# NVIDIA-RTX/RTXPT

Hardware: AMD Instinct MI355X
Metric: Mrays/s at 4K 4spp 8-bounce bistro-like (extend + shadow rays / wall time of pt_render) (higher is better)
Workload: dtype f32; 1 GPU; C3 bistro-like street canyon, 2808008 triangles, 64 materials, 32 textures 1024^2, 7368 emissive-triangle + env-quad lights, 3840x2160, 4 spp, 8 bounces, NEE 5 candidates + RR, lp types binary16 (reference default), environment cube 2048 BC6H (reference default on D3D12); BVH builder=PLOC + parallel re-insertion + cost-driven wide nodes, built on device, buildMs 78.6 (host part 0.0), 275780 wide n; parallelism=pixel-tile shard x1 + 1 gather, gather=none (1 GPU), transport=none, rehearsal=False

## Files before the change

### include/mi355pt_testhooks.h

```cpp
#ifndef MI355PT_TESTHOOKS_H
#define MI355PT_TESTHOOKS_H
#include "mi355pt.h"
#ifdef __cplusplus
extern "C" {
#endif
int32_t pt_probe(pt_context* ctx, int32_t kind, const void* in, size_t inBytes, void* out, size_t outBytes, uint32_t n);
#ifdef __cplusplus
}
#endif
#endif
```

### rtxpt_amd/__init__.py

```python
import ctypes
import os
import subprocess

import numpy as np

from . import scenes

_HERE = os.path.dirname(os.path.abspath(__file__))
LIB_PATH = os.environ.get("MI355PT_LIB", os.path.join(_HERE, "libmi355pt.so"))
HOOKS_LIB_PATH = os.path.join(_HERE, "libmi355pt_testhooks.so")
_libs = {}

PT_OK = 0
PT_ERROR_INVALID_ARGUMENT, PT_ERROR_NO_DEVICE, PT_ERROR_HIP, PT_ERROR_IO, PT_ERROR_UNSUPPORTED, PT_ERROR_NOT_READY = 1, 2, 3, 4, 5, 6
PT_TEX_RGBA8_UNORM, PT_TEX_RGBA8_SRGB, PT_TEX_RGBA32F = 0, 1, 2
STATUS = {0: "PT_OK", 1: "PT_ERROR_INVALID_ARGUMENT", 2: "PT_ERROR_NO_DEVICE", 3: "PT_ERROR_HIP", 4: "PT_ERROR_IO", 5: "PT_ERROR_UNSUPPORTED", 6: "PT_ERROR_NOT_READY"}

EXPORTS = [
    "pt_create", "pt_destroy", "pt_get_last_error", "pt_load_scene_gltf", "pt_gltf_animation_load", "pt_gltf_animation_instances", "pt_gltf_animation_positions", "pt_gltf_animation_normals", "pt_animate_normals", "pt_gltf_animation_free", "pt_set_geometry", "pt_set_instances", "pt_set_materials",
    "pt_set_environment", "pt_set_environment_cube", "pt_image_read_dds_cube", "pt_set_environment_bake", "pt_set_environment_compression", "pt_set_procedural_sky", "pt_procedural_sky_default_params", "pt_procedural_sky_update", "pt_env_bake_lights", "pt_set_lights", "pt_set_light_importance_boost", "pt_set_local_light_sampling", "pt_get_light_feedback", "pt_set_neeat", "pt_set_view_projection", "pt_neeat_reset", "pt_get_neeat_tables", "pt_neeat_pack_feedback", "pt_neeat_unpack_feedback", "pt_bridge_camera", "pt_set_camera", "pt_default_settings", "pt_set_settings", "pt_animate",
    "pt_resize", "pt_render", "pt_reset_accumulation", "pt_map_radiance", "pt_unmap_radiance", "pt_shard_info", "pt_pack_shard",
    "pt_unpack_shard", "pt_device_radiance", "pt_trace_closest", "pt_trace_visibility", "pt_get_lights", "pt_get_env_cube", "pt_get_subinstances",
    "pt_get_scene_info", "pt_get_build_stats", "pt_get_bvh_info", "pt_set_counters",
    "pt_default_tonemap", "pt_tonemap", "pt_image_read_float", "pt_image_free", "pt_image_read_dds", "pt_image_read_dds_memory", "pt_image_read_jpeg", "pt_scene_import_texture", "pt_write_png", "pt_write_bmp", "pt_set_fused_traversal", "pt_set_serial_kernels", "pt_set_tail_paths", "pt_animate_ranges", "pt_set_motion_history", "pt_set_previous_pose", "pt_realtime_frame", "pt_exchange_planes_host", "pt_neeat_update_begin", "pt_neeat_update_end", "pt_pack_stable_plane_guides", "pt_unpack_stable_plane_guides", "pt_stable_planes_shard_bytes", "pt_pack_stable_planes", "pt_unpack_stable_planes", "pt_gather_stable_planes", "pt_material_from_json", "pt_convert_light",
    "pt_tonemap_color_transform", "pt_scene_json_import", "pt_scene_import_free", "pt_scene_import_cameras", "pt_scene_import_lights",
    "pt_scene_import_directional_lights", "pt_scene_import_instances", "pt_scene_import_geometries", "pt_scene_import_materials", "pt_scene_import_vertices", "pt_set_scene_directional_lights", "pt_scene_import_apply", "pt_scene_import_settings", "pt_average_luminance",
    "pt_default_tone_mapping_parameters", "pt_tonemap_from_parameters", "pt_scene_import_tone_mapping",
    "pt_stable_planes_plane_stride", "pt_build_stable_planes", "pt_fill_stable_planes", "pt_denoise_spec_hit_t", "pt_stable_planes_merge", "pt_get_stable_planes",
    "pt_denoiser_default_params", "pt_denoiser_prepare_dlss_rr", "pt_denoiser_prepare_nrd", "pt_denoiser_merge_nrd", "pt_get_denoiser_inputs", "pt_denoiser_device_buffers",
    "pt_denoise_default_settings", "pt_denoise_plane", "pt_denoised_device_buffers", "pt_get_denoised", "pt_denoise_frame", "pt_denoise_pass_times",
    "pt_taa_default_params", "pt_taa_resolve", "pt_resolved_device_buffer", "pt_get_resolved", "pt_tonemap_resolved", "pt_taa_jitter",
    "pt_bloom_default_params", "pt_bloom_kernel", "pt_bloom", "pt_bloomed_device_buffer", "pt_get_bloomed", "pt_tonemap_bloomed", "pt_average_luminance_bloomed",
    "pt_taa_upscale_default_params", "pt_taa_upscale", "pt_upscaled_size", "pt_upscaled_device_buffer", "pt_get_upscaled", "pt_bloom_upscaled", "pt_get_upscaled_bloomed",
    "pt_tonemap_upscaled", "pt_average_luminance_upscaled", "pt_upscale_tex_lod_bias",
    "pt_comm_unique_id", "pt_comm_init", "pt_comm_destroy", "pt_gather", "pt_shard_layout", "pt_gather_host", "pt_neeat_exchange_host",
]
TEST_HOOK_EXPORTS = ["pt_probe"]


class PtError(RuntimeError):
    def __init__(self, code, msg=""):
        super().__init__("%s (%d): %s" % (STATUS.get(code, "?"), code, msg))
        self.code = code


class PtGeometryBuffers(ctypes.Structure):
    _fields_ = [("indices", ctypes.c_void_p), ("numIndices", ctypes.c_uint32), ("positions", ctypes.c_void_p), ("uvs", ctypes.c_void_p),
                ("normals", ctypes.c_void_p), ("tangents", ctypes.c_void_p), ("numVertices", ctypes.c_uint32)]


class PtTextureDesc(ctypes.Structure):
    _fields_ = [("width", ctypes.c_uint32), ("height", ctypes.c_uint32), ("format", ctypes.c_uint32), ("pixels", ctypes.c_void_p)]


class PtEnvMapSceneParams(ctypes.Structure):
    _fields_ = [("Transform", ctypes.c_float * 12), ("ColorMultiplier", ctypes.c_float * 3), ("Enabled", ctypes.c_float)]


class PtProceduralSkyConstants(ctypes.Structure):
    _fields_ = [("StarIrradiance", ctypes.c_float * 3), ("StarAngularDiameter", ctypes.c_float), ("RayleightScatteringRGB", ctypes.c_float * 3), ("PlanetSurfaceRadius", ctypes.c_float),
                ("MieScatteringRGB", ctypes.c_float * 3), ("PlanetAtmosphereRadius", ctypes.c_float), ("MieHenyeyGreensteinG", ctypes.c_float), ("SqDistanceToHorizontalBoundary", ctypes.c_float),
                ("AtmosphereHeight", ctypes.c_float), ("reserved", ctypes.c_float),
                ("FinalRadianceMultiplier", ctypes.c_float * 3), ("_padding3", ctypes.c_float), ("SunDir", ctypes.c_float * 3), ("CloudsTime", ctypes.c_float),
                ("GroundAlbedo", ctypes.c_float * 3), ("SunAngularDiameter", ctypes.c_float), ("_padding0", ctypes.c_float), ("_padding1", ctypes.c_float), ("sun_solid_angle", ctypes.c_float),
                ("_padding2", ctypes.c_float), ("physical_sky_ground_radiance", ctypes.c_float * 3), ("cloud_density_offset", ctypes.c_float),
                ("sky_transmittance", ctypes.c_float), ("sky_phase_g", ctypes.c_float), ("sky_amb_phase_g", ctypes.c_float), ("sky_scattering", ctypes.c_float)]

    def as_array(self): return np.frombuffer(bytes(self), np.float32).copy()


class PtSkyTexture(ctypes.Structure):
    _fields_ = [("rgba", ctypes.c_void_p), ("width", ctypes.c_uint32), ("height", ctypes.c_uint32), ("depth", ctypes.c_uint32), ("_pad", ctypes.c_uint32)]


class PtProceduralSkyTextures(ctypes.Structure):
    _fields_ = [("transmittance", PtSkyTexture), ("scattering", PtSkyTexture), ("irradiance", PtSkyTexture), ("clouds", PtSkyTexture)]


class PtProceduralSkyParams(ctypes.Structure):
    _fields_ = [("colorTint", ctypes.c_float * 3), ("brightness", ctypes.c_float), ("sunBrightness", ctypes.c_float), ("cloudsMovementSpeed", ctypes.c_float), ("timeOfDayMovementSpeed", ctypes.c_float),
                ("sunTimeOfDayOffset", ctypes.c_float), ("sunEastWestRotation", ctypes.c_float), ("sunAngularDiameterDeg", ctypes.c_float), ("cloudDensityOffset", ctypes.c_float),
                ("cloudTransmittance", ctypes.c_float), ("cloudScattering", ctypes.c_float)]


class PtProceduralSkyState(ctypes.Structure):
    _fields_ = [("lastSceneTime", ctypes.c_double), ("timeOfDayL1", ctypes.c_float), ("timeOfDayL2", ctypes.c_float), ("lastConstants", PtProceduralSkyConstants)]


def _sky_textures(textures):
    keep, t = [], PtProceduralSkyTextures()
# ... 1118 lines not shown

    def lights(self):
        n, npx, dim = ctypes.c_uint32(), ctypes.c_uint32(), ctypes.c_uint32()
        self._chk(self.L.pt_get_lights(self.h, ctypes.byref(n), ctypes.byref(npx), None, None, None, None, None, ctypes.byref(dim)), "pt_get_lights")
        lights = np.zeros((n.value, 8), np.uint32)
        ex = np.zeros((n.value, 4), np.uint32)
        pc = np.zeros(n.value, np.uint32)
        pi = np.zeros(npx.value, np.uint32)
        el = np.zeros(dim.value * dim.value, np.uint32)
        self._chk(self.L.pt_get_lights(self.h, None, None, _p(lights), _p(ex), _p(pc), _p(pi), _p(el), None), "pt_get_lights")
        return dict(lights=lights, lightsEx=ex, proxyCounters=pc, proxyIndices=pi, envLookup=el, envLookupDim=dim.value)

    def env_cube(self):
        n, dim, lv = ctypes.c_uint32(), ctypes.c_uint32(), ctypes.c_uint32()
        self._chk(self.L.pt_get_env_cube(self.h, ctypes.byref(n), ctypes.byref(dim), ctypes.byref(lv), None, 0), "pt_get_env_cube")
        out = np.zeros((n.value, 2), np.uint32)
        if n.value: self._chk(self.L.pt_get_env_cube(self.h, None, None, None, _p(out), n.value), "pt_get_env_cube")
        return out, dim.value, lv.value

    def subinstances(self):
        n = ctypes.c_uint32()
        self._chk(self.L.pt_get_subinstances(self.h, ctypes.byref(n), None), "pt_get_subinstances")
        out = np.zeros((n.value, 8), np.uint32)
        self._chk(self.L.pt_get_subinstances(self.h, None, _p(out)), "pt_get_subinstances")
        return out

    def scene_info(self):
        a, b, c, d = ctypes.c_uint32(), ctypes.c_uint32(), ctypes.c_uint32(), ctypes.c_uint32()
        self._chk(self.L.pt_get_scene_info(self.h, ctypes.byref(a), ctypes.byref(b), ctypes.byref(c), ctypes.byref(d)), "pt_get_scene_info")
        return dict(triangles=a.value, bvhNodes=b.value, instances=c.value, materials=d.value)

    def build_stats(self):
        a, b, c = ctypes.c_double(), ctypes.c_double(), ctypes.c_double()
        self._chk(self.L.pt_get_build_stats(self.h, ctypes.byref(a), ctypes.byref(b), ctypes.byref(c)), "pt_get_build_stats")
        return dict(buildMs=a.value, refitMs=b.value, lightBakeMs=c.value)

    def bvh_info(self):
        class PtBvhInfo(ctypes.Structure):
            _fields_ = [("builder", ctypes.c_uint32), ("builtOnDevice", ctypes.c_uint32), ("numTriangles", ctypes.c_uint32), ("numWideNodes", ctypes.c_uint32),
                        ("collapseLevels", ctypes.c_uint32), ("optimiserPasses", ctypes.c_uint32), ("hostMs", ctypes.c_float), ("buildMs", ctypes.c_float)]
        o = PtBvhInfo()
        self._chk(self.L.pt_get_bvh_info(self.h, ctypes.byref(o)), "pt_get_bvh_info")
        names = {0: "PLOC", 1: "Karras radix tree", 2: "binned SAH + re-insertion (host)", 3: "PLOC + parallel re-insertion + cost-driven wide nodes"}
        d = {k: getattr(o, k) for k, _ in PtBvhInfo._fields_}
        d["builderName"] = names.get(o.builder, "?"); d["builtOn"] = "device" if o.builtOnDevice else "host"
        return d

    def probe(self, kind, inp, out_shape, out_dtype=np.float32):
        if not self.test_hooks: raise RuntimeError("pt_probe is not part of the shipped library: PathTracer(test_hooks=True)")
        inp = np.ascontiguousarray(inp)
        out = np.zeros(out_shape, out_dtype)
        self._chk(self.L.pt_probe(self.h, kind, _p(inp), inp.nbytes, _p(out), out.nbytes, out_shape[0]), "pt_probe")
        return out
```

### rtxpt_amd/csrc/pt_api.hip

```cpp
#include <cstring>
#include <rocprim/rocprim.hpp>
#include "pt_context.h"
#ifdef MI355PT_TEST_HOOKS
#include "../../include/mi355pt_testhooks.h"
#endif
#include "pt_denoiser.h"
#include <dlfcn.h>
#include <algorithm>
#include <cmath>
#include <cstdio>
#include <chrono>

using namespace ptk;

static_assert(sizeof(::PTMaterialData) == sizeof(ptk::PTMaterialData), "material ABI");
static_assert(sizeof(::PathTracerCameraData) == sizeof(ptk::PathTracerCameraData), "camera ABI");
static_assert(sizeof(::PtSettings) == sizeof(ptk::PtSettings), "settings ABI");
static_assert(sizeof(::PtGeometryDesc) == sizeof(ptk::GeometryDesc), "geometry ABI");
static_assert(sizeof(::PtInstanceDesc) == sizeof(ptk::InstanceDesc), "instance ABI");
static_assert(sizeof(::PolymorphicLightInfo) == sizeof(ptk::PolymorphicLightInfo), "light ABI");

namespace {

void build_mips(HostTexture& t) {
// ... 134 lines not shown
    PT_CHECK_HIP(c, c->dPrevPositions.resize(c->positions.size())); PT_CHECK_HIP(c, c->dPrevInstances.resize(c->instances.size()));
    if (c->instances.size()) PT_CHECK_HIP(c, hipMemcpyAsync(c->dPrevInstances.p, c->dInstances.p, sizeof(InstanceDesc) * c->instances.size(), hipMemcpyDeviceToDevice, c->stream));
    if (fresh || c->prevAllStale) { if (c->positions.size()) PT_CHECK_HIP(c, hipMemcpyAsync(c->dPrevPositions.p, c->dPositions.p, 4 * c->positions.size(), hipMemcpyDeviceToDevice, c->stream)); }
    else for (size_t r = 0; r + 1 < c->prevStaleRanges.size(); r += 2) {
        const size_t first = 3 * (size_t)c->prevStaleRanges[r], count = 3 * (size_t)c->prevStaleRanges[r + 1];
        if (count) PT_CHECK_HIP(c, hipMemcpyAsync(c->dPrevPositions.p + first, c->dPositions.p + first, 4 * count, hipMemcpyDeviceToDevice, c->stream));
    }
    c->prevAllStale = false; c->prevStaleRanges.clear();
    return PT_OK;
}
int finalize_geometry(pt_context* c) {
    c->subInstances.clear(); c->subInstToInstGeom.clear(); c->primInfo.clear(); c->subInstFirstPrim.clear();
    for (size_t i = 0; i < c->instances.size(); i++) {
        if (c->instances[i].meshIndex >= c->meshes.size()) return fail(c, PT_ERROR_INVALID_ARGUMENT, "instance references a missing mesh");
        const MeshDesc& m = c->meshes[c->instances[i].meshIndex];
        for (uint g = 0; g < m.numGeometries; g++) {
            uint gi = m.firstGeometry + g;
            if (gi >= c->geometries.size()) return fail(c, PT_ERROR_INVALID_ARGUMENT, "mesh references a missing geometry");
            const GeometryDesc& gd = c->geometries[gi];
            if (gd.materialIndex >= c->materials.size()) return fail(c, PT_ERROR_INVALID_ARGUMENT, "geometry references a missing material");
            const ptk::PTMaterialData& mat = c->materials[gd.materialIndex];
            SubInstanceData si; memset(&si, 0, sizeof(si));
            bool alphaTested = (gd.geomFlags & GEOMF_ALPHA_TESTED) && (mat.Flags & PTMaterialFlags_UseBaseOrDiffuseTexture) && (gd.flags & GEOM_HAS_UV);
            if (alphaTested) {
                si.FlagsAndAlphaInfo |= SubInstanceData::Flags_AlphaTested;
                uint cutoff = (uint)(saturate(mat.AlphaCutoff) * 255.0f);
                si.FlagsAndAlphaInfo |= (cutoff & 0xFFu) << SubInstanceData::Flags_AlphaOffsetOffset;
                si.FlagsAndAlphaInfo |= (mat.BaseOrDiffuseTextureIndex & 0xFFFFu);
            }
            if (gd.geomFlags & GEOMF_EXCLUDE_FROM_NEE) si.FlagsAndAlphaInfo |= SubInstanceData::Flags_ExcludeFromNEE;
            si.GlobalGeometryIndex_PTMaterialDataIndex = (gi << 16) | (gd.materialIndex & 0xFFFFu);
            si.EmissiveLightMappingOffset = 0xFFFFFFFFu; si.AnalyticProxyLightIndex = 0xFFFFFFFFu;
            si.IndexOffset = gd.indexOffset; si.TexCoord1Offset = gd.vertexOffset;
            uint subInst = (uint)c->subInstances.size();
            c->subInstToInstGeom.push_back(ptk::make_uint2((uint)i, gi));
            c->subInstances.push_back(si); c->subInstFirstPrim.push_back((uint)c->primInfo.size());
            for (uint t = 0; t < gd.numIndices / 3; t++) c->primInfo.push_back(ptk::make_uint2(subInst, t));
        }
    }
    if (c->primInfo.size() > 0x7FFFFFFull / 3ull * 2ull)
        return fail(c, PT_ERROR_UNSUPPORTED, "more than 89 M triangles per scene are not supported by the traversal kernels");
    c->numTris = (uint)c->primInfo.size();
    hipStream_t st = c->stream;
    PT_CHECK_HIP(c, c->dIndices.upload(c->indices, st)); PT_CHECK_HIP(c, c->dPositions.upload(c->positions, st)); PT_CHECK_HIP(c, c->dUvs.upload(c->uvs, st));
    PT_CHECK_HIP(c, c->dNormals.upload(c->normals, st)); PT_CHECK_HIP(c, c->dTangents.upload(c->tangents, st));
    PT_CHECK_HIP(c, c->dGeometries.upload(c->geometries, st)); PT_CHECK_HIP(c, c->dInstances.upload(c->instances, st));
    PT_CHECK_HIP(c, c->dSubInstances.upload(c->subInstances, st)); PT_CHECK_HIP(c, c->dSubInstToInstGeom.upload(c->subInstToInstGeom, st));
    PT_CHECK_HIP(c, c->dPrimInfo.upload(c->primInfo, st)); PT_CHECK_HIP(c, c->dMaterials.upload(c->materials, st));
    if (c->motionHistory) { c->prevAllStale = true; c->prevStaleRanges.clear(); int r = motion_history_sync(c); if (r != PT_OK) return r; }
    if (c->bvhAllocated && c->bvh.capacity < c->numTris) { bvh_free(c->bvh); c->bvhAllocated = false; }
    if (!c->bvhAllocated) { PT_CHECK_HIP(c, bvh_alloc(c->bvh, c->numTris)); c->bvhAllocated = true; }
    c->bvh.builder = c->bvhBuilder;
    { const char* e = getenv("MI355PT_REINSERT_PASSES"); c->bvh.riPasses = e ? (uint)atoi(e) : 12u; }
    PT_CHECK_HIP(c, c->dShadeTris.resize(c->numTris));
    if (!c->dTravSpill.p) PT_CHECK_HIP(c, c->dTravSpill.resize(PT_PIPELINE_BATCHES * (size_t)T8_MAX_BLOCKS * T8_GROUPS_PER_BLOCK * T8_SPILL_DEPTH));
    refresh_scene_view(c);
    hipEvent_t e0, e1; PT_CHECK_HIP(c, hipEventCreate(&e0)); PT_CHECK_HIP(c, hipEventCreate(&e1));
    PT_CHECK_HIP(c, hipEventRecord(e0, st));
    PT_CHECK_HIP(c, bvh_build(c->bvh, c->dsc, c->numTris, st));
    PT_CHECK_HIP(c, hipEventRecord(e1, st));
    launch_shade_tris(c->dsc, 0u, c->numTris, c->dShadeTris.p, st);
    PT_CHECK_HIP(c, hipStreamSynchronize(st));
    float ms = 0; (void)hipEventElapsedTime(&ms, e0, e1); c->buildMs = ms; (void)hipEventDestroy(e0); (void)hipEventDestroy(e1);
    c->geomDirty = false; c->lightsDirty = true;
    return PT_OK;
}

const uint RTXPT_LIGHTING_MAX_LIGHTS = 512 * 1024, RTXPT_LIGHTING_SAMPLING_PROXY_RATIO = 12, RTXPT_LIGHTING_MAX_SAMPLING_PROXIES_PER_LIGHT = 256 * 1024;
const float RTXPT_LIGHTING_MIN_WEIGHT_THRESHOLD = 1e-8f;
const uint QT_BASE_RES = 4, QT_SUBDIV = 24, QT_UNBOOSTED = QT_BASE_RES * QT_BASE_RES + 3 * QT_SUBDIV, QT_BOOST_DPT = 3, QT_BOOST_SUBDIV = 20,
           QT_BOOST_MULT = QT_BOOST_SUBDIV * 3 + 1, QT_TOTAL = QT_UNBOOSTED * QT_BOOST_MULT, EMISB_DIM = 1024;
struct EnvImportance { uint dim, mipCount; std::vector<std::vector<ptk::float4>> mips; };
uint firstbithigh(uint v) { uint r = 0; while (v >>= 1) r++; return r; }
uint qt_weight(const EnvImportance& im, uint dim, uint x, uint y, uint lightIndex, uint depthLimit) {
    uint mipLevel = im.mipCount - firstbithigh(dim) - 1;
    float areaMul = (float)(1u << (mipLevel * 2));
    float radiance = im.mips[mipLevel][(size_t)y * dim + x].w;
    float ret = areaMul * radiance;
    ret = fmaxf_(sq(1.0f / 100.0f) * (float)mipLevel, ret);
    ret *= (mipLevel > depthLimit) ? 1.0f : 0.0f;
    uint v = (uint)(FastSqrt(ret) * 100 + 0.5f); if (v > 0x000FFFFFu) v = 0x000FFFFFu;
    return (v << 12) | lightIndex;
}
struct QTNode { uint dim, x, y; };
void qt_subdivide(const EnvImportance& im, std::vector<QTNode>& nodes, std::vector<uint>& packed, uint subdivisions, uint depthLimit) {
    for (uint si = 0; si < subdivisions; si++) {
        uint best = 0; for (size_t i = 0; i < packed.size(); i++) best = std::max(best, packed[i]);
        uint gi = best & 0xFFFu;
        QTNode n = nodes[gi];
        for (uint k = 0; k < 4; k++) {
            QTNode ch; ch.dim = n.dim * 2; ch.x = n.x * 2 + (k % 2); ch.y = n.y * 2 + (k / 2);
            uint ni = (k == 0) ? gi : (uint)nodes.size();
            if (k == 0) { nodes[gi] = ch; packed[gi] = qt_weight(im, ch.dim, ch.x, ch.y, ni, depthLimit); }
            else { nodes.push_back(ch); packed.push_back(qt_weight(im, ch.dim, ch.x, ch.y, ni, depthLimit)); }
        }
    }
}
int bake_env_quads(pt_context* c) {
    EnvImportance im; im.dim = EMISB_DIM; im.mipCount = 11; im.mips.resize(im.mipCount);
    PT_CHECK_HIP(c, c->dScratch4.resize((size_t)im.dim * im.dim));
    launch_env_importance(c->dsc, im.dim, 4, 4, c->dScratch4.p, c->stream);
    im.mips[0].resize((size_t)im.dim * im.dim);
    PT_CHECK_HIP(c, hipMemcpyAsync(im.mips[0].data(), c->dScratch4.p, sizeof(ptk::float4) * im.mips[0].size(), hipMemcpyDeviceToHost, c->stream));
    PT_CHECK_HIP(c, hipStreamSynchronize(c->stream));
    for (uint l = 1; l < im.mipCount; l++) {
        uint pd = im.dim >> (l - 1), d = im.dim >> l;
        im.mips[l].resize((size_t)d * d);
        const std::vector<ptk::float4>& p = im.mips[l - 1];
        for (uint y = 0; y < d; y++) for (uint x = 0; x < d; x++) {
            ptk::float4 s = (p[(size_t)(2 * y) * pd + 2 * x] + p[(size_t)(2 * y) * pd + 2 * x + 1]) + (p[(size_t)(2 * y + 1) * pd + 2 * x] + p[(size_t)(2 * y + 1) * pd + 2 * x + 1]);
            im.mips[l][(size_t)y * d + x] = ptk::env_round_rgba16f(s * 0.25f);
        }
    }
    std::vector<QTNode> base; std::vector<uint> packed;
// ... 48 lines not shown
}
int bake_lights(pt_context* c, bool geometryOnly = false) {
    hipEvent_t e0, e1; PT_CHECK_HIP(c, hipEventCreate(&e0)); PT_CHECK_HIP(c, hipEventCreate(&e1));
    PT_CHECK_HIP(c, hipEventRecord(e0, c->stream));
    const bool keepEnv = geometryOnly && c->S.NEEEnabled && c->envEnabled && c->envLightsBaked == QT_TOTAL && c->lights.size() >= QT_TOTAL;
    if (!keepEnv) { c->lights.clear(); c->lightsEx.clear(); c->envLookup.clear(); c->envLookupDim = 0; c->envLightsBaked = 0; }
    else { c->lights.resize(QT_TOTAL); c->lightsEx.resize(QT_TOTAL); }
    c->numProxies = 0;
    for (auto& si : c->subInstances) { si.EmissiveLightMappingOffset = 0xFFFFFFFFu; si.AnalyticProxyLightIndex = 0xFFFFFFFFu; }
    if (c->S.NEEEnabled) {
        if (c->envEnabled && !keepEnv) { c->lights.resize(QT_TOTAL); c->lightsEx.resize(QT_TOTAL); int r = bake_env_quads(c); if (r != PT_OK) return r; c->envLightsBaked = QT_TOTAL; }
        const uint analyticBase = (uint)c->lights.size();
        for (auto& a : c->analyticLights) { c->lights.push_back(a.Base); c->lightsEx.push_back(a.Extended); }
        for (size_t s = 0; s < c->subInstances.size(); s++) {
            const uint proxy = c->instances[c->subInstToInstGeom[s].x].analyticProxyLight;
            if (proxy && proxy <= c->analyticLights.size() && (c->materials[c->subInstances[s].GlobalGeometryIndex_PTMaterialDataIndex & 0xFFFFu].Flags & PTMaterialFlags_EnableAsAnalyticLightProxy))
                c->subInstances[s].AnalyticProxyLightIndex = analyticBase + proxy - 1u;
        }
        std::vector<uint> list, offsets; uint total = 0; uint lightBase = (uint)c->lights.size();
        for (size_t s = 0; s < c->subInstances.size(); s++) {
            const GeometryDesc& g = c->geometries[c->subInstances[s].GlobalGeometryIndex_PTMaterialDataIndex >> 16];
            const ptk::PTMaterialData& mat = c->materials[g.materialIndex];
            bool isEmissive = any_gt0(mat.EmissiveColor);
            uint ntri = g.numIndices / 3;
            if (!isEmissive || (size_t)lightBase + total + ntri >= RTXPT_LIGHTING_MAX_LIGHTS) continue;
            c->subInstances[s].EmissiveLightMappingOffset = lightBase + total;
            list.push_back((uint)s); offsets.push_back(total); total += ntri;
        }
        c->lights.resize((size_t)lightBase + total); c->lightsEx.resize((size_t)lightBase + total);
        const uint N = (uint)c->lights.size();
        PT_CHECK_HIP(c, c->dLights.resize(N)); PT_CHECK_HIP(c, c->dLightsEx.resize(N));
        if (lightBase && !keepEnv) {
            PT_CHECK_HIP(c, hipMemcpyAsync(c->dLights.p, c->lights.data(), sizeof(ptk::PolymorphicLightInfo) * lightBase, hipMemcpyHostToDevice, c->stream));
            PT_CHECK_HIP(c, hipMemcpyAsync(c->dLightsEx.p, c->lightsEx.data(), sizeof(ptk::PolymorphicLightInfoEx) * lightBase, hipMemcpyHostToDevice, c->stream));
        } else if (keepEnv && lightBase > QT_TOTAL) {
            PT_CHECK_HIP(c, hipMemcpyAsync(c->dLights.p + QT_TOTAL, c->lights.data() + QT_TOTAL, sizeof(ptk::PolymorphicLightInfo) * (lightBase - QT_TOTAL), hipMemcpyHostToDevice, c->stream));
            PT_CHECK_HIP(c, hipMemcpyAsync(c->dLightsEx.p + QT_TOTAL, c->lightsEx.data() + QT_TOTAL, sizeof(ptk::PolymorphicLightInfoEx) * (lightBase - QT_TOTAL), hipMemcpyHostToDevice, c->stream));
        }
        if (total) {
            PT_CHECK_HIP(c, c->dEmissiveList.upload(list, c->stream)); PT_CHECK_HIP(c, c->dEmissiveOffsets.upload(offsets, c->stream));
            launch_bake_emissive(c->dsc, c->dEmissiveList.p, c->dEmissiveOffsets.p, (uint)list.size(), total, lightBase, c->dLights.p, c->dLightsEx.p, c->stream);
        }
        if (N) {
            const uint budget = RTXPT_LIGHTING_SAMPLING_PROXY_RATIO * std::max(N, RTXPT_LIGHTING_MAX_LIGHTS / 10);
            const size_t proxyCapacity = (size_t)budget + N;
            (void)budget; (void)proxyCapacity;
            PT_CHECK_HIP(c, c->dLightW.resize(N + 1));
            launch_light_weights(c->dLights.p, c->dLightsEx.p, N, c->dLightW.p, c->lightBoost, c->stream);
            int pr = build_light_proxies(c, c->dLightW.p, nullptr, 0u, 0.f); if (pr != PT_OK) return pr;
        }
    } else { PT_CHECK_HIP(c, c->dLights.resize(1)); PT_CHECK_HIP(c, c->dLightsEx.resize(1)); }
    if (!keepEnv) PT_CHECK_HIP(c, c->dEnvLookup.upload(c->envLookup, c->stream));
    PT_CHECK_HIP(c, c->dSubInstances.upload(c->subInstances, c->stream));
    PT_CHECK_HIP(c, hipEventRecord(e1, c->stream));
    PT_CHECK_HIP(c, hipStreamSynchronize(c->stream));
    float ms = 0; (void)hipEventElapsedTime(&ms, e0, e1); c->lightBakeMs = ms; (void)hipEventDestroy(e0); (void)hipEventDestroy(e1);
    refresh_scene_view(c);
    c->lightsDirty = false;
    return PT_OK;
}
int bake_env_cube(pt_context* c) {
    ptk::EnvCube& e = c->envCube; memset(&e, 0, sizeof(e)); e.dim = c->envCubeDim; e.mipLevels = ptk::env_cube_mip_levels(e.dim);
    size_t total = 0; for (uint l = 0; l < e.mipLevels; l++) { e.mipOffset[l] = (uint)total; total += 6ull * (e.dim >> l) * (e.dim >> l); }
    PT_CHECK_HIP(c, c->dEnvCube.resize(total));
    std::vector<ptk::EnvDirectionalLight> dirLights = c->envDirLights;
    if (!c->sceneDirLights.empty()) {
        PtEnvMapSceneParams prm; memset(&prm, 0, sizeof(prm)); memcpy(prm.Transform, c->envToWorld.m, 48); prm.Enabled = 1.f;
        std::vector<ptk::EnvDirectionalLight> conv(c->sceneDirLights.size());
        if (pt_env_bake_lights(reinterpret_cast<const PtEnvDirectionalLight*>(c->sceneDirLights.data()), (uint32_t)conv.size(), &prm, e.dim, reinterpret_cast<PtEnvDirectionalLight*>(conv.data())) != PT_OK) return fail(c, PT_ERROR_INVALID_ARGUMENT, "scene directional lights");
        for (auto& l : conv) if (dirLights.size() < 16u) dirLights.push_back(l);
    }
    PT_CHECK_HIP(c, c->dEnvDirLights.upload(dirLights, c->stream));
    if (c->skyEnabled) {
        ptk::ProceduralSkyContext h = c->sky; h.Transmittance.texels = c->dSkyTex[0].p; h.Scatter.texels = c->dSkyTex[1].p; h.Irradiance.texels = c->dSkyTex[2].p; h.Clouds.texels = c->dSkyTex[3].p;
        PT_CHECK_HIP(c, c->dSky.resize(1)); PT_CHECK_HIP(c, hipMemcpyAsync(c->dSky.p, &h, sizeof(h), hipMemcpyHostToDevice, c->stream)); PT_CHECK_HIP(c, hipStreamSynchronize(c->stream));
        PT_CHECK_HIP(c, c->dSkyLowRes.resize(6ull * (e.dim / 2u) * (e.dim / 2u)));
    }
    refresh_scene_view(c);
    launch_env_cube_bake(c->dsc, c->dEnvDirLights.p, (uint)dirLights.size(), c->dEnvCube.p, c->dsc.envCube, c->stream);
    if (c->envCompression) {
        PT_CHECK_HIP(c, c->dEnvCubeSource.resize(total));
        PT_CHECK_HIP(c, hipMemcpyAsync(c->dEnvCubeSource.p, c->dEnvCube.p, sizeof(ptk::uint2) * total, hipMemcpyDeviceToDevice, c->stream));
        launch_env_cube_compress(c->dEnvCube.p, c->dsc.envCube, c->envCompression, c->stream);
    } else c->dEnvCubeSource.free();
    refresh_scene_view(c);
    PT_CHECK_HIP(c, hipGetLastError());
    c->envCubeDirty = false; c->lightsDirty = true;
    return PT_OK;
}
}

int prepare(pt_context* c) {
    if (c->texDirty) { int r = upload_textures(c); if (r != PT_OK) return r; refresh_scene_view(c); c->lightsDirty = true; c->envCubeDirty = true; }
    if (c->envEnabled && c->envCubeDirty) { int r = bake_env_cube(c); if (r != PT_OK) return r; }
    if (c->geomDirty) { int r = finalize_geometry(c); if (r != PT_OK) return r; }
    if (c->lightsDirty) { int r = bake_lights(c); if (r != PT_OK) return r; }
    else if (c->weightsDirty && !c->lights.empty()) {
        launch_light_weights(c->dLights.p, c->dLightsEx.p, (uint)c->lights.size(), c->dLightW.p, c->lightBoost, c->stream);
        int r = build_light_proxies(c, c->dLightW.p, nullptr, 0u, 0.f); if (r != PT_OK) return r;
        refresh_scene_view(c);
    }
    c->weightsDirty = false;
    return PT_OK;
}

int neeat_exchange_feedback(pt_context* c) {
// ... 54 lines not shown
    F.updateCounter = st.updateCounter; F.dropoff = st.dropoff; F.totalLightCount = N; F.historicTotalLightCount = st.framePrevLightCount;
    F.lastFrameFeedbackAvailable = lastFrameFeedbackAvailable ? 1u : 0u; F.lastFrameLocalSamplesAvailable = (lastFrameLocalSamplesAvailable && lastFrameFeedbackAvailable) ? 1u : 0u;
    F.fbW = st.fbW.p; F.fbC = st.fbC.p; F.scW = st.scW.p; F.scC = st.scC.p; F.blW = st.blW.p; F.blC = st.blC.p; F.local = st.local.p;
    F.depth = depth ? depth : st.depth.p; F.motion = motion; F.historyDepth = st.histDepth.p; F.depthDisocclusionThreshold = 1.5f;
    const uint totalMaxFeedbackCount = lastFrameFeedbackAvailable ? ((F.W + 7) / 8) * ((F.H + 7) / 8) * 64u : 0u;
    if (phases & NEEAT_BEGIN) {
        PT_CHECK_HIP(c, st.counters.resize(N + 1)); PT_CHECK_HIP(c, hipMemsetAsync(st.counters.p, 0, 4 * (size_t)(N + 1), c->stream)); F.perLightCounters = st.counters.p;
        if (lastFrameFeedbackAvailable) launch_neeat_begin(F, st.snapW.p, st.snapC.p, st.preFilter, totalMaxFeedbackCount, c->stream);
        PT_CHECK_HIP(c, st.curW.resize(N + 1)); PT_CHECK_HIP(c, st.histW.resize(N));
        launch_neeat_boost_weights(c->dLightW.p, (lastFrameFeedbackAvailable && st.intensityDeltaMul > 0) ? st.histW.p : nullptr, st.nHist, N, st.intensityDeltaMul, st.curW.p, c->stream);
        int r = build_light_proxies(c, st.curW.p, lastFrameFeedbackAvailable ? st.counters.p : nullptr, totalMaxFeedbackCount, lastFrameFeedbackAvailable ? st.globalFeedbackWeight : 0.f); if (r != PT_OK) return r;
        PT_CHECK_HIP(c, hipMemcpyAsync(st.histW.p, st.curW.p, 4 * (size_t)N, hipMemcpyDeviceToDevice, c->stream)); st.nHist = N;
        st.lastFeedbackAvailable = lastFrameFeedbackAvailable;
    }
    if (!(phases & NEEAT_END)) { PT_CHECK_HIP(c, hipStreamSynchronize(c->stream)); return PT_OK; }
    F.perLightCounters = st.counters.p;
    F.samplingProxyCount = c->numProxies; F.proxies = c->dProxyIndices.p;
    launch_neeat_end(F, c->stream);
    if (!depth) PT_CHECK_HIP(c, hipMemsetAsync(st.depth.p, 0, 4 * px, c->stream));
    st.exportDepth = depth == nullptr;
    st.feedbackFilled = true; st.frameOpen = false;
    c->localResX = F.tilesX; c->localResY = F.tilesY; c->localJitterX = st.jitter[0]; c->localJitterY = st.jitter[1]; c->localMaxLight = 0;
    c->localRatio = lastFrameFeedbackAvailable ? st.localRatio : 0.f; c->sscThreshold = st.sscThreshold; c->feedbackRequired = true;
    refresh_scene_view(c);
    PT_CHECK_HIP(c, hipStreamSynchronize(c->stream));
    return PT_OK;
}

extern "C" {

int32_t pt_create(const PtDeviceDesc* desc, pt_context** out) {
    if (!out) return PT_ERROR_INVALID_ARGUMENT;
    *out = nullptr;
    int ndev = 0;
    if (hipGetDeviceCount(&ndev) != hipSuccess || ndev <= 0) return PT_ERROR_NO_DEVICE;
    int dev = desc ? desc->deviceOrdinal : 0;
    if (dev < 0 || dev >= ndev) return PT_ERROR_INVALID_ARGUMENT;
    if (hipSetDevice(dev) != hipSuccess) return PT_ERROR_HIP;
    pt_context* c = new pt_context();
    c->device = dev; c->shardRank = desc ? desc->shardRank : 0; c->shardCount = (desc && desc->shardCount) ? desc->shardCount : 1;
    if (c->shardRank >= c->shardCount) { delete c; return PT_ERROR_INVALID_ARGUMENT; }
    if (hipStreamCreateWithFlags(&c->stream, hipStreamNonBlocking) != hipSuccess) { delete c; return PT_ERROR_HIP; }
    c->streams[0] = c->stream;
    for (uint b = 1; b < PT_PIPELINE_BATCHES; b++) if (hipStreamCreateWithFlags(&c->streams[b], hipStreamNonBlocking) != hipSuccess) { delete c; return PT_ERROR_HIP; }
    if (hipHostMalloc(&c->hostCounters, PT_PIPELINE_BATCHES * sizeof(WaveCounters), hipHostMallocDefault) != hipSuccess) { delete c; return PT_ERROR_HIP; }
    c->serialKernels = desc && (desc->flags & PT_DEVICE_SERIAL_KERNELS);
    c->bvhBuilder = (desc && (desc->flags & PT_DEVICE_PREFER_FAST_BUILD)) ? BVH_BUILDER_PLOC : ((desc && (desc->flags & PT_DEVICE_HOST_SAH_BUILDER)) ? BVH_BUILDER_SAH : BVH_BUILDER_PLOC_OPT);
    { const char* e = getenv("MI355PT_BVH_BUILDER");
      if (e && !strcmp(e, "karras")) c->bvhBuilder = BVH_BUILDER_KARRAS; else if (e && !strcmp(e, "ploc")) c->bvhBuilder = BVH_BUILDER_PLOC; else if (e && !strcmp(e, "sah")) c->bvhBuilder = BVH_BUILDER_SAH; else if (e && (!strcmp(e, "ploc_opt") || !strcmp(e, "device"))) c->bvhBuilder = BVH_BUILDER_PLOC_OPT; }
    { const char* e = getenv("MI355PT_TAIL_PATHS"); if (e) c->tailBelow = (uint)strtoul(e, nullptr, 10); }
    { const char* e = getenv("MI355PT_COMPACT_POOL"); if (e) c->compactPool = atoi(e) != 0; }
    { const char* e = getenv("MI355PT_FIRST_VERTEX_IN_PLACE"); if (e) c->firstVertexInPlace = atoi(e) != 0; }
    { const char* e = getenv("MI355PT_FUSED_TRAVERSAL"); if (e) c->fusedTraversal = (uint)strtoul(e, nullptr, 10); }
    { const char* e = getenv("MI355PT_TAIL_DEFER"); if (e) c->tailDefer = (uint)strtoul(e, nullptr, 10); }
    memset(&c->dsc, 0, sizeof(c->dsc)); memset(&c->cam, 0, sizeof(c->cam)); memset(&c->bvh, 0, sizeof(c->bvh));
    pt_default_settings(reinterpret_cast<::PtSettings*>(&c->S));
    const float I[12] = {1, 0, 0, 0, 0, 1, 0, 0, 0, 0, 1, 0}; memcpy(c->envToWorld.m, I, 48); memcpy(c->envToLocal.m, I, 48); c->envColorMul = ptk::make_float3(1.0f / ptk::kEnvMapRadianceScale);
    if (c->dCounters.resize(PT_PIPELINE_BATCHES) != hipSuccess) { delete c; return PT_ERROR_HIP; }
    *out = c;
    return PT_OK;
}
int32_t pt_destroy(pt_context* c) {
    if (!c) return PT_ERROR_INVALID_ARGUMENT;
    (void)hipSetDevice(c->device); (void)hipStreamSynchronize(c->stream);
    if (c->comm && g_rccl.lib) { (void)g_rccl.CommDestroy(c->comm); c->comm = nullptr; }
    c->dSpHeader.free(); c->dSpThroughput.free(); c->dSpPlanes.free(); c->dSpRadiance.free(); c->dSpMotion.free(); c->dSpDepth.free(); c->dSpHitT.free(); c->dSpMark.free(); c->dSpNewL.free(); c->dSpScratch.free(); c->dSpGatherSend.free(); c->dSpGatherRecv.free(); c->dSpGatherPixels.free();
    c->dDnRRDiff.free(); c->dDnRRSpec.free(); c->dDnRRSpecMV.free(); c->dDnRRNormal.free(); c->dDnMotion.free(); c->dDnViewZ.free(); c->dDnRoughness.free(); c->dDnNormal.free(); c->dDnDiff.free(); c->dDnSpec.free(); c->dDnDisocclusion.free(); c->dDnHistoryClamp.free();
    relax_free(c); taa_free(c); bloom_free(c); taau_free(c);
    c->neeat.free(); c->dLocalTable.free(); c->dFbWeight.free(); c->dFbCand.free(); c->dSq3.free();
    c->dGatherSend.free(); c->dGatherRecv.free(); c->dGatherPixels.free(); c->dLightW.free(); c->dProxyOffsets.free(); if (c->dScanTemp) (void)hipFree(c->dScanTemp);
    if (c->bvhAllocated) bvh_free(c->bvh);
    c->dIndices.free(); c->dNormals.free(); c->dTangents.free(); c->dProxyCounters.free(); c->dProxyIndices.free(); c->dEnvLookup.free(); c->dOwned.free(); c->dQueue[0].free(); c->dQueue[1].free();
    c->dPrevPositions.free(); c->dPrevInstances.free(); c->dEmissiveList.free(); c->dEmissiveOffsets.free(); c->dPositions.free(); c->dUvs.free(); c->dGeometries.free(); c->dInstances.free(); c->dSubInstances.free(); c->dSubInstToInstGeom.free();
    c->dPrimInfo.free(); c->dShadeTris.free(); c->dAlphaPlanes.free(); c->dAlphaPool.free(); c->dMaterials.free(); c->dTexInfos.free(); c->dTexels.free(); c->dEnvCube.free(); c->dEnvCubeSource.free(); c->dEnvImageCube.free(); c->dEnvDirLights.free(); c->dLights.free(); c->dLightsEx.free(); c->dS0.free(); c->dS1.free(); c->dS2.free(); c->dS3.free(); c->dS4.free();
    c->dHit.free(); c->dS0b.free(); c->dS1b.free(); c->dS3b.free(); c->dS4b.free(); c->dHitb.free(); c->dSq0.free(); c->dSq1.free(); c->dSq2.free(); c->dAccum.free(); c->dScratch4.free(); c->dCounters.free(); c->dTravSpill.free(); c->dTaskQ.free(); c->dTravCounts.free(); c->dResolveList.free(); c->dBestKey.free(); c->dResolveListSh.free(); c->dBestKeySh.free(); c->dTaskQSh.free();
    for (uint b = 1; b < PT_PIPELINE_BATCHES; b++) (void)hipStreamDestroy(c->streams[b]);
    (void)hipStreamDestroy(c->stream); (void)hipHostFree(c->hostCounters);
    delete c;
    return PT_OK;
}
const char* pt_get_last_error(pt_context* c) { return c ? c->lastError.c_str() : "null context"; }

int32_t pt_set_geometry(pt_context* c, const PtGeometryBuffers* b, const PtGeometryDesc* geoms, uint32_t nGeoms, const PtMeshDesc* meshes, uint32_t nMeshes) {
    if (!c || !b || !geoms || !meshes) return fail(c, PT_ERROR_INVALID_ARGUMENT, "null argument");
    if (!b->indices || !b->positions) return fail(c, PT_ERROR_INVALID_ARGUMENT, "indices and positions are required");
    for (uint32_t g = 0; g < nGeoms; g++) {
        if ((size_t)geoms[g].indexOffset + geoms[g].numIndices > b->numIndices || (size_t)geoms[g].vertexOffset + geoms[g].numVertices > b->numVertices || geoms[g].numIndices % 3)
            return fail(c, PT_ERROR_INVALID_ARGUMENT, "geometry range outside the supplied streams");
        if ((geoms[g].flags & PT_GEOM_HAS_UV) && !b->uvs) return fail(c, PT_ERROR_INVALID_ARGUMENT, "geometry has uv flag but no uv stream");
        if ((geoms[g].flags & PT_GEOM_HAS_NORMAL) && !b->normals) return fail(c, PT_ERROR_INVALID_ARGUMENT, "geometry has normal flag but no normal stream");
        if ((geoms[g].flags & PT_GEOM_HAS_TANGENT) && !b->tangents) return fail(c, PT_ERROR_INVALID_ARGUMENT, "geometry has tangent flag but no tangent stream");
        const uint32_t* idx = b->indices + geoms[g].indexOffset;
        for (uint32_t k = 0; k < geoms[g].numIndices; k++) if (idx[k] >= geoms[g].numVertices) return fail(c, PT_ERROR_INVALID_ARGUMENT, "index outside the geometry's vertex range");
    }
    for (uint32_t m = 0; m < nMeshes; m++)
        if ((size_t)meshes[m].firstGeometry + meshes[m].numGeometries > nGeoms) return fail(c, PT_ERROR_INVALID_ARGUMENT, "mesh references geometries outside the supplied array");
    uint nv = b->numVertices;
    c->indices.assign(b->indices, b->indices + b->numIndices);
    c->positions.assign(b->positions, b->positions + 3 * (size_t)nv);
    c->uvs.assign(nv, ptk::make_float2(0, 0)); if (b->uvs) memcpy(c->uvs.data(), b->uvs, 8 * (size_t)nv);
    c->normals.assign(nv, 0); if (b->normals) memcpy(c->normals.data(), b->normals, 4 * (size_t)nv);
    c->tangents.assign(nv, 0); if (b->tangents) memcpy(c->tangents.data(), b->tangents, 4 * (size_t)nv);
    c->geometries.resize(nGeoms); memcpy(c->geometries.data(), geoms, sizeof(GeometryDesc) * nGeoms);
    c->meshes.resize(nMeshes); memcpy(c->meshes.data(), meshes, sizeof(MeshDesc) * nMeshes);
    c->geomDirty = true;
    relax_drop_history(c); taa_drop_history(c); taau_drop_history(c);
    return PT_OK;
}
int32_t pt_set_instances(pt_context* c, const PtInstanceDesc* inst, uint32_t n) {
    if (!c || (!inst && n)) return fail(c, PT_ERROR_INVALID_ARGUMENT, "null argument");
    c->instances.resize(n); if (n) memcpy(c->instances.data(), inst, sizeof(InstanceDesc) * n);
    c->geomDirty = true;
    return PT_OK;
}
int32_t pt_set_materials(pt_context* c, const ::PTMaterialData* mats, uint32_t nMats, const PtTextureDesc* tex, uint32_t nTex) {
    if (!c || (!mats && nMats) || (!tex && nTex)) return fail(c, PT_ERROR_INVALID_ARGUMENT, "null argument");
    c->materials.resize(nMats); if (nMats) memcpy(c->materials.data(), mats, 128 * (size_t)nMats);
    c->textures.clear();
    for (uint32_t i = 0; i < nTex; i++) {
        const PtTextureDesc& d = tex[i];
        if (!d.pixels || !d.width || !d.height || d.format > 2) return fail(c, PT_ERROR_INVALID_ARGUMENT, "bad texture descriptor");
        if (d.width > 32768u || d.height > 32768u) return fail(c, PT_ERROR_UNSUPPORTED, "textures above 32768 texels per side are not supported (16 mip levels)");
        HostTexture t; t.w = d.width; t.h = d.height; t.mips.resize(1); t.mips[0].resize((size_t)d.width * d.height);
        for (size_t k = 0; k < (size_t)d.width * d.height; k++) {
            ptk::float4 v;
            if (d.format == PT_TEX_RGBA32F) { const float* p = (const float*)d.pixels + 4 * k; v = ptk::make_float4(p[0], p[1], p[2], p[3]); }
            else {
// ... 777 lines not shown
}
int32_t pt_get_env_cube(pt_context* c, uint32_t* texelCount, uint32_t* dim, uint32_t* mipLevels, void* texels8B, uint32_t capacityTexels) {
    if (!c) return PT_ERROR_INVALID_ARGUMENT;
    (void)hipSetDevice(c->device);
    int r = prepare(c); if (r != PT_OK) return r;
    size_t n = 0;
    if (c->envEnabled) { const uint last = c->envCube.mipLevels - 1u, d = c->envCube.dim >> last; n = (size_t)c->envCube.mipOffset[last] + 6ull * d * d; }
    if (texelCount) *texelCount = (uint32_t)n; if (dim) *dim = c->envEnabled ? c->envCube.dim : 0; if (mipLevels) *mipLevels = c->envEnabled ? c->envCube.mipLevels : 0;
    if (texels8B && n) {
        if (capacityTexels < n) return fail(c, PT_ERROR_INVALID_ARGUMENT, "pt_get_env_cube: buffer too small");
        PT_CHECK_HIP(c, hipStreamSynchronize(c->stream));
        PT_CHECK_HIP(c, hipMemcpy(texels8B, c->dEnvCube.p, 8 * n, hipMemcpyDeviceToHost));
    }
    return PT_OK;
}
int32_t pt_get_subinstances(pt_context* c, uint32_t* count, void* out) {
    if (!c) return PT_ERROR_INVALID_ARGUMENT;
    (void)hipSetDevice(c->device);
    int r = prepare(c); if (r != PT_OK) return r;
    if (count) *count = (uint32_t)c->subInstances.size();
    if (out && c->subInstances.size()) PT_CHECK_HIP(c, hipMemcpy(out, c->dSubInstances.p, 32 * c->subInstances.size(), hipMemcpyDeviceToHost));
    return PT_OK;
}
int32_t pt_get_scene_info(pt_context* c, uint32_t* nTris, uint32_t* nNodes, uint32_t* nInst, uint32_t* nMat) {
    if (!c) return PT_ERROR_INVALID_ARGUMENT;
    (void)hipSetDevice(c->device);
    int r = prepare(c); if (r != PT_OK) return r;
    if (nTris) *nTris = c->numTris; if (nNodes) *nNodes = c->numTris ? c->bvh.numNodes8 : 0;       if (nInst) *nInst = (uint32_t)c->instances.size(); if (nMat) *nMat = (uint32_t)c->materials.size();
    return PT_OK;
}
#ifdef MI355PT_TEST_HOOKS
int32_t pt_probe(pt_context* c, int32_t kind, const void* in, size_t inBytes, void* out, size_t outBytes, uint32_t n) {
    if (!c || !in || !out || !n) return fail(c, PT_ERROR_INVALID_ARGUMENT, "bad argument");
    (void)hipSetDevice(c->device);
    if (kind == 8 || kind == 9 || kind == 10 || kind == 11) { int r = prepare(c); if (r != PT_OK) return r; }
    if (kind == 11) {
        if (inBytes < (size_t)n * 32u || outBytes < (size_t)n * 16u) return fail(c, PT_ERROR_INVALID_ARGUMENT, "texture probe: 8 words in and 4 floats out per row");
        const uint32_t* a = (const uint32_t*)in;
        for (uint32_t i = 0; i < n; i++, a += 8) {
            const uint32_t tex = a[0] == 0u ? (a[1] & 0xFFFFu) : a[1];
            if (a[0] > 2u || tex >= c->textures.size() || (a[0] == 1u && a[4] >= c->textures[tex].mipLevels)) return fail(c, PT_ERROR_INVALID_ARGUMENT, "texture probe: mode, texture or mip out of range");
        }
    }
    DevBuf<unsigned char> di, dout;
    PT_CHECK_HIP(c, di.upload((const unsigned char*)in, inBytes, c->stream)); PT_CHECK_HIP(c, dout.resize(outBytes));
    PathKernelContext k; k.sc = c->dsc; k.S = c->S; k.cam = c->cam;
    launch_probe(k, kind, di.p, dout.p, n, c->stream);
    PT_CHECK_HIP(c, hipMemcpyAsync(out, dout.p, outBytes, hipMemcpyDeviceToHost, c->stream));
    PT_CHECK_HIP(c, hipStreamSynchronize(c->stream));
    PT_CHECK_HIP(c, hipGetLastError());
    di.free(); dout.free();
    return PT_OK;
}
#endif
int32_t pt_shard_layout(uint32_t width, uint32_t height, uint32_t rank, uint32_t world, uint32_t* pixels, uint32_t capacity, uint32_t* count) {
    if (!width || !height || width > 65535 || height > 65535 || !world || rank >= world) return PT_ERROR_INVALID_ARGUMENT;
    std::vector<std::vector<uint>> lists; shard_pixel_lists(width, height, world, lists);
    const std::vector<uint>& mine = lists[rank];
    if (count) *count = (uint32_t)mine.size();
    if (pixels) { if (capacity < mine.size()) return PT_ERROR_INVALID_ARGUMENT; if (!mine.empty()) memcpy(pixels, mine.data(), 4 * mine.size()); }
    return PT_OK;
}
int32_t pt_comm_unique_id(void* id128) {
    if (!id128) return PT_ERROR_INVALID_ARGUMENT;
    if (!g_rccl.load()) return PT_ERROR_HIP;
    static_assert(sizeof(ncclUniqueId) == PT_COMM_ID_BYTES, "unique id size");
    ncclUniqueId id; if (g_rccl.GetUniqueId(&id) != ncclSuccess) return PT_ERROR_HIP;
    memcpy(id128, &id, sizeof(id));
    return PT_OK;
}
int32_t pt_comm_init(pt_context* c, const void* id128, uint32_t rank, uint32_t world) {
    if (!c || !id128) return fail(c, PT_ERROR_INVALID_ARGUMENT, "null argument");
    if (rank != c->shardRank || world != c->shardCount) return fail(c, PT_ERROR_INVALID_ARGUMENT, "pt_comm_init: rank / world must equal the context's shardRank / shardCount");
    if (!g_rccl.load()) return fail(c, PT_ERROR_HIP, g_rccl.error);
    (void)hipSetDevice(c->device);
    if (c->comm) { (void)g_rccl.CommDestroy(c->comm); c->comm = nullptr; }
    ncclUniqueId id; memcpy(&id, id128, sizeof(id));
    PT_CHECK_NCCL(c, g_rccl.CommInitRank(&c->comm, (int)world, id, (int)rank));
    c->commRank = rank; c->commWorld = world; c->gatherW = c->gatherH = 0;
    return PT_OK;
}
int32_t pt_comm_destroy(pt_context* c) {
    if (!c) return PT_ERROR_INVALID_ARGUMENT;
    if (c->comm && g_rccl.lib) { (void)hipSetDevice(c->device); (void)hipStreamSynchronize(c->stream); (void)g_rccl.CommDestroy(c->comm); }
    c->comm = nullptr;
    return PT_OK;
}
int32_t pt_gather(pt_context* c) {
    if (!c) return PT_ERROR_INVALID_ARGUMENT;
    if (!c->width) return fail(c, PT_ERROR_NOT_READY, "pt_resize first");
    if (c->shardCount == 1 && !c->comm) return PT_OK;
    if (!c->comm) return fail(c, PT_ERROR_NOT_READY, "pt_comm_init first");
    (void)hipSetDevice(c->device);
    hipStream_t st = c->stream;
    if (c->shardCount == 1) {
        const size_t n = c->owned.size();
        if (!n) return PT_OK;
        PT_CHECK_HIP(c, c->dGatherSend.resize(n)); PT_CHECK_HIP(c, c->dGatherRecv.resize(n));
        launch_pack(c->dAccum.p, c->dOwned.p, (uint)n, c->width, c->dGatherSend.p, st);
        PT_CHECK_HIP(c, hipMemsetAsync(c->dAccum.p, 0xFF, sizeof(ptk::float4) * (size_t)c->width * c->height, st));
        PT_CHECK_NCCL(c, g_rccl.GroupStart());
        ncclResult_t rs = g_rccl.Send(c->dGatherSend.p, 4 * n, ncclFloat, 0, c->comm, st);
        ncclResult_t rr = (rs == ncclSuccess) ? g_rccl.Recv(c->dGatherRecv.p, 4 * n, ncclFloat, 0, c->comm, st) : rs;
        ncclResult_t re = g_rccl.GroupEnd();
        if (rr != ncclSuccess || re != ncclSuccess) return fail(c, PT_ERROR_HIP, std::string("pt_gather loop-back: ") + g_rccl.GetErrorString(rr != ncclSuccess ? rr : re));
        launch_unpack(c->dAccum.p, c->dOwned.p, (uint)n, c->width, c->dGatherRecv.p, st);
// ... 116 lines not shown
```

### rtxpt_amd/csrc/pt_build.h

```cpp
#pragma once
#include "pt_scene.h"
#include <hip/hip_runtime.h>

namespace ptk {

enum : uint { BVH_BUILDER_PLOC = 0, BVH_BUILDER_KARRAS = 1, BVH_BUILDER_SAH = 2, BVH_BUILDER_PLOC_OPT = 3 };

struct TriSrc { uint instance, i0, i1, i2, prim, flags, _pad0, _pad1; };
static const uint BVH_MAX_WIDE_LEVELS = 64;

struct BvhBuildBuffers {
    TriRecord* triWorld;
    TriRecord* triSorted;
    unsigned long long* keys; unsigned long long* keysSorted;
    uint* prims; uint* primsSorted;
    uint* childL; uint* childR; uint* parent; uint* leafParent; uint* rangeFirst; uint* rangeLast;
    uint* tickets;
    float4* boxLmin; float4* boxLmax; float4* boxRmin; float4* boxRmax;
    uint* sceneBounds;
    BvhNode* nodes;
    AlphaRec* alphaRecs;
    float4* rangeMin; float4* rangeMax; uint rangeLevels;
    uint* primToSlot;
    Bvh8Node* nodes8; uint* levelA; uint* levelB; uint* wideCounter; uint numNodes8, collapseLevels;
    TriSrc* triSrc;
    float4* wideBoxMin; float4* wideBoxMax;
    uint wideLevelStart[BVH_MAX_WIDE_LEVELS + 1]; uint wideRefitReady;
    bool bvh2Stale = false;
    void* sortTemp; size_t sortTempBytes;
    uint* plocCl[2]; uint* plocNN; unsigned long long* plocFlags; unsigned long long* plocOffs; uint* plocChildA; uint* plocChildB; uint* plocCnt; uint* plocParent; uint* plocFirst; uint* plocCounts;
    void* scanTemp; size_t scanTempBytes; uint plocPasses;
    uint builder;
    uint* absorb;
    float hostBuildMs;
    void* riScratch; size_t riScratchBytes; uint riPasses, riLevels;
    uint wideDpPending;
    uint wideFlagsValid;
    uint wideLevels;
    uint optimiserPasses;
    uint capacity;
};

hipError_t bvh_alloc(BvhBuildBuffers& b, uint numTris);
void bvh_free(BvhBuildBuffers& b);
hipError_t bvh_build(BvhBuildBuffers& b, const DeviceScene& sc, uint numTris, hipStream_t stream);
void launch_shade_tris(const DeviceScene& sc, uint firstPrim, uint numTris, ShadeTri* out, hipStream_t stream);
hipError_t bvh_refit(BvhBuildBuffers& b, const DeviceScene& sc, uint numTris, hipStream_t stream);

}
```

### rtxpt_amd/csrc/pt_build.hip

```cpp
#include "pt_build.h"
#include "pt_build_sah.h"
#include "pt_build_wide.h"
#include "pt_build_reinsert.h"
#include <chrono>
#include <cstdlib>
#include <vector>
#include <rocprim/rocprim.hpp>

#ifndef PT_PLOC_RADIUS
#define PT_PLOC_RADIUS 32
#endif
#ifndef PT_RANGE_TABLE_MAX_TRIS
#define PT_RANGE_TABLE_MAX_TRIS (16u << 20)
#endif

namespace ptk {

#define PT_HIP_TRY(x) do { hipError_t e_ = (x); if (e_ != hipSuccess) return e_; } while (0)

__device__ __forceinline__ uint enc_float(float f) { uint b = __float_as_uint(f); return (b & 0x80000000u) ? ~b : (b | 0x80000000u); }
__device__ __forceinline__ float dec_float(uint u) { uint b = (u & 0x80000000u) ? (u & 0x7FFFFFFFu) : ~u; return __uint_as_float(b); }

__device__ __forceinline__ float wave_min(float v) { for (int o = 32; o > 0; o >>= 1) v = fminf(v, __shfl_xor(v, o)); return v; }
__device__ __forceinline__ float wave_max(float v) { for (int o = 32; o > 0; o >>= 1) v = fmaxf(v, __shfl_xor(v, o)); return v; }
// ... 428 lines not shown
    uint q0 = 0x00FFFFFFu, q1 = 0u;
    if (valid) bvh8_child_codes(mn, mx, nmn, sx, sy, sz, q0, q1);
    nd[4u + 3u * k] = valid ? r : BVH_EMPTY; nd[5u + 3u * k] = q0; nd[6u + 3u * k] = q1;
    if (k == 0u) { nd[0] = __float_as_uint(nmn.x); nd[1] = __float_as_uint(nmn.y); nd[2] = __float_as_uint(nmn.z); nd[3] = ex | (ey << 8) | (ez << 16) | (n << 24); }
    if (k == 1u) { nd[28] = __float_as_uint(sx); nd[29] = __float_as_uint(sy); nd[30] = __float_as_uint(sz); nd[31] = 0u; }
}

__global__ void __launch_bounds__(256) k_alpha_records(DeviceScene sc, const TriRecord* __restrict__ triSorted, uint n, AlphaRec* __restrict__ recs, uint* __restrict__ primToSlot) {
    uint i = blockIdx.x * 256u + threadIdx.x;
    if (i >= n) return;
    primToSlot[triSorted[i].prim] = i;
    AlphaRec r; r.t0 = r.t1 = r.t2 = make_float2(0.f, 0.f); r.tex = 0xFFFFFFFFu; r.cutoff = 0.f; r.wh = r.plane = r.fmt = r._pad = 0u;
    TriRecord tr = triSorted[i];
    if (tr.flags & 1u) {
        uint2 pi = sc.primInfo[tr.prim];
        const SubInstanceData& si = sc.subInstances[pi.x];
        if (si.FlagsAndAlphaInfo & SubInstanceData::Flags_AlphaTested) {
            const uint* idx = sc.indices + si.IndexOffset + pi.y * 3;
            r.t0 = sc.uvs[si.TexCoord1Offset + idx[0]]; r.t1 = sc.uvs[si.TexCoord1Offset + idx[1]]; r.t2 = sc.uvs[si.TexCoord1Offset + idx[2]];
            r.tex = si.AlphaTextureIndex(); r.cutoff = si.AlphaCutoff();
            const AlphaPlane ap = sc.alphaPlanes[r.tex]; r.wh = ap.wh; r.plane = ap.offset; r.fmt = ap.fmt;
        }
    }
    recs[i] = r;
}

__global__ void __launch_bounds__(256) k_shade_tris(DeviceScene sc, uint firstPrim, uint numTris, ShadeTri* __restrict__ out) {
    uint p = blockIdx.x * 256u + threadIdx.x;
    if (p >= numTris) return;
    p += firstPrim;
    const uint2 pi = sc.primInfo[p];
    const uint2 ig = sc.subInstToInstGeom[pi.x];
    const GeometryDesc& g = sc.geometries[ig.y];
    const uint* idx = sc.indices + g.indexOffset + 3u * pi.y;
    const uint v0 = g.vertexOffset + idx[0], v1 = g.vertexOffset + idx[1], v2 = g.vertexOffset + idx[2];
    const float* P = sc.positions;
    ShadeTri r; __builtin_memset(&r, 0, sizeof(r));
    r.instance = ig.x; r.subInstance = pi.x; r.triangleIndex = pi.y;
    r.materialAndFlags = (sc.subInstances[pi.x].GlobalGeometryIndex_PTMaterialDataIndex & 0xFFFFu) | (g.flags << 16);
    r.p0 = make_float3(P[3 * v0], P[3 * v0 + 1], P[3 * v0 + 2]); r.p1 = make_float3(P[3 * v1], P[3 * v1 + 1], P[3 * v1 + 2]); r.p2 = make_float3(P[3 * v2], P[3 * v2 + 1], P[3 * v2 + 2]);
    if (g.flags & GEOM_HAS_UV) { r.t0 = sc.uvs[v0]; r.t1 = sc.uvs[v1]; r.t2 = sc.uvs[v2]; }
    if (g.flags & GEOM_HAS_NORMAL) {
        const float3 objFlatN = SafeNormalize(cross(r.p1 - r.p0, r.p2 - r.p0));
        const uint pn[3] = {sc.normals[v0], sc.normals[v1], sc.normals[v2]}; float3 n[3];
        for (int k = 0; k < 3; k++) { n[k] = normalize(Unpack_RGB8_SNORM(pn[k])); if (dot(n[k], objFlatN) < 0.f) n[k] = -n[k]; }
        r.n0 = n[0]; r.n1 = n[1]; r.n2 = n[2];
    }
    if (g.flags & GEOM_HAS_TANGENT) { r.g0 = sc.tangents[v0]; r.g1 = sc.tangents[v1]; r.g2 = sc.tangents[v2]; }
    uint4* o = reinterpret_cast<uint4*>(out + p); const uint4* src = reinterpret_cast<const uint4*>(&r);
    for (int k = 0; k < 8; k++) o[k] = src[k];
}
void launch_shade_tris(const DeviceScene& sc, uint firstPrim, uint numTris, ShadeTri* out, hipStream_t st) {
    if (numTris) hipLaunchKernelGGL(k_shade_tris, dim3((numTris + 255u) / 256u), dim3(256), 0, st, sc, firstPrim, numTris, out);
}

__global__ void __launch_bounds__(256) k_wide_levels(const uint* __restrict__ levelIn, uint nIn, const uint* __restrict__ childL, const uint* __restrict__ childR,
                                                     const uint* __restrict__ rangeFirst, const uint* __restrict__ rangeLast, uint maxLeaf, uint* __restrict__ levelOut, uint* __restrict__ counter) {
    __shared__ uint sCnt[4]; __shared__ uint sBase;
    const uint i = blockIdx.x * 256u + threadIdx.x, wave = threadIdx.x >> 6, lane = threadIdx.x & 63u;
    uint kids[2]; uint nk = 0;
    if (i < nIn) {
        const uint id = levelIn[i];
        if (rangeLast[id] - rangeFirst[id] + 1u > maxLeaf) {
            const uint L = childL[id], R = childR[id];
            if (!(L & BVH_LEAF_BIT)) kids[nk++] = L;
            if (!(R & BVH_LEAF_BIT)) kids[nk++] = R;
        }
    }
    const unsigned long long m1 = __builtin_amdgcn_ballot_w64(nk >= 1u), m2 = __builtin_amdgcn_ballot_w64(nk >= 2u), below = (1ull << lane) - 1ull;
    const uint inWave = (uint)__popcll(m1 & below) + (uint)__popcll(m2 & below);
    if (lane == 0u) sCnt[wave] = (uint)__popcll(m1) + (uint)__popcll(m2);
    __syncthreads();
    if (threadIdx.x == 0u) { uint tot = 0; for (uint w = 0; w < 4u; w++) { const uint c = sCnt[w]; sCnt[w] = tot; tot += c; } sBase = tot ? atomicAdd(counter, tot) : 0u; }
    __syncthreads();
    const uint at = sBase + sCnt[wave] + inWave;
    for (uint k = 0; k < nk; k++) levelOut[at + k] = kids[k];
}
__global__ void __launch_bounds__(256) k_wide_dp(const uint* __restrict__ level, uint nIn, const uint* __restrict__ childL, const uint* __restrict__ childR, const uint* __restrict__ rangeFirst,
                                                 const uint* __restrict__ rangeLast, uint maxLeaf, const float4* __restrict__ boxLmin, const float4* __restrict__ boxLmax,
                                                 const float4* __restrict__ boxRmin, const float4* __restrict__ boxRmax, float* __restrict__ C, unsigned long long* __restrict__ dec) {
    const uint i = blockIdx.x * 256u + threadIdx.x; if (i >= nIn) return;
    const uint id = level[i];
    const float4 a = boxLmin[id], b = boxLmax[id], c = boxRmin[id], d = boxRmax[id];
    const float lmn[3] = {a.x, a.y, a.z}, lmx[3] = {b.x, b.y, b.z}, rmn[3] = {c.x, c.y, c.z}, rmx[3] = {d.x, d.y, d.z};
    wide_dp_node(id, childL[id], childR[id], rangeLast[id] - rangeFirst[id] + 1u, maxLeaf, lmn, lmx, rmn, rmx, C, dec);
}
__global__ void __launch_bounds__(256) k_wide_mark(const uint* __restrict__ level, uint nIn, const uint* __restrict__ childL, const uint* __restrict__ childR, const uint* __restrict__ rangeFirst,
                                                   const uint* __restrict__ rangeLast, uint maxLeaf, const unsigned long long* __restrict__ dec, uint* __restrict__ absorb, uint* __restrict__ state) {
    const uint i = blockIdx.x * 256u + threadIdx.x; if (i >= nIn) return;
    const uint id = level[i];
    wide_mark_node(id, state[id], childL[id], childR[id], rangeLast[id] - rangeFirst[id] + 1u, maxLeaf, dec, absorb, state);
}
static hipError_t bvh_wide_nodes(BvhBuildBuffers& b, uint n, hipStream_t st) {
    if (n < 2u || !b.rangeMin) return hipErrorInvalidValue;
    uint* order = b.levelA; uint* state = b.levelB; float* C = reinterpret_cast<float*>(b.rangeMin); unsigned long long* dec = b.plocFlags;
    PT_HIP_TRY(hipMemsetAsync(b.absorb, 0, 4 * (size_t)n, st)); PT_HIP_TRY(hipMemsetAsync(state, 0, 4 * (size_t)n, st));
    const uint first[2] = {0u, wide_state(8u, true)};
    PT_HIP_TRY(hipMemcpyAsync(order, &first[0], 4, hipMemcpyHostToDevice, st)); PT_HIP_TRY(hipMemcpyAsync(state, &first[1], 4, hipMemcpyHostToDevice, st));
    std::vector<uint> start{0u}, count{1u};
    for (;;) {
        const uint s0 = start.back(), c0 = count.back();
        if ((size_t)s0 + c0 > n) return hipErrorUnknown;
        PT_HIP_TRY(hipMemsetAsync(b.wideCounter, 0, 4, st));
        hipLaunchKernelGGL(k_wide_levels, dim3((c0 + 255u) / 256u), dim3(256), 0, st, order + s0, c0, b.childL, b.childR, b.rangeFirst, b.rangeLast, BVH_MAX_LEAF, order + s0 + c0, b.wideCounter);
        uint next = 0; PT_HIP_TRY(hipMemcpyAsync(&next, b.wideCounter, 4, hipMemcpyDeviceToHost, st)); PT_HIP_TRY(hipStreamSynchronize(st));
        if (!next) break;
// ... 316 lines not shown
```

### rtxpt_amd/csrc/pt_context.h

```cpp
#pragma once
#include "../../include/mi355pt.h"
#include "pt_wavefront.h"
#include "pt_stableplanes_launch.h"
#include "pt_denoiser.h"
#include "pt_build.h"
#include <rccl/rccl.h>
#include <string>
#include <vector>

#pragma GCC visibility push(hidden)

using namespace ptk;

template <typename T> struct DevBuf {
    T* p = nullptr; size_t n = 0;
    hipError_t resize(size_t count) {
        if (count <= n && p) return hipSuccess;
        if (p) (void)hipFree(p);
        p = nullptr; n = 0;
        hipError_t e = hipMalloc(&p, sizeof(T) * (count ? count : 1));
        if (e == hipSuccess) n = count ? count : 1;
        return e;
    }
    hipError_t upload(const T* src, size_t count, hipStream_t st) {
        hipError_t e = resize(count); if (e != hipSuccess) return e;
        if (!count) return hipSuccess;
        return hipMemcpyAsync(p, src, sizeof(T) * count, hipMemcpyHostToDevice, st);
    }
    hipError_t upload(const std::vector<T>& v, hipStream_t st) { return upload(v.data(), v.size(), st); }
    void free() { if (p) (void)hipFree(p); p = nullptr; n = 0; }
};

struct HostTexture { uint w, h, mipLevels; std::vector<std::vector<ptk::float4>> mips; };

static const uint TILE = 32;
static const uint TASK_QUEUE_CAPACITY = 1u << 22;
#ifndef PT_SHARD_TILE_GROUP
#define PT_SHARD_TILE_GROUP 1
#endif
#ifndef PT_PIPELINE_FULL_AT
#define PT_PIPELINE_FULL_AT (1u << 21)
#endif
#ifndef PT_PIPELINE_MID_BATCHES
#define PT_PIPELINE_MID_BATCHES 2
#endif
#ifndef PT_CLASSIFY_FROM
#define PT_CLASSIFY_FROM 65536u
#endif
#ifndef PT_SP_FILL_CLASSES
#define PT_SP_FILL_CLASSES 1
#endif
#ifndef PT_SP_FILL_RANGED
#define PT_SP_FILL_RANGED 1
#endif
#ifndef PT_TAIL_PATHS
#define PT_TAIL_PATHS 4096u
#endif
#ifndef PT_FUSED_TRAVERSAL
#define PT_FUSED_TRAVERSAL 1u
#endif
#ifndef PT_FUSED_BELOW
#define PT_FUSED_BELOW (12u << 20)
#endif
#ifndef PT_COMPACT_POOL
#define PT_COMPACT_POOL 1
#endif
#ifndef PT_FIRST_VERTEX_IN_PLACE
#define PT_FIRST_VERTEX_IN_PLACE 1
#endif
#ifndef PT_FREE_RUN_BELOW
#define PT_FREE_RUN_BELOW (1u << 22)
#endif
#ifndef PT_PIPELINE_BATCHES
#define PT_PIPELINE_BATCHES 4
#endif

#pragma GCC visibility pop
struct pt_context {
    int device = 0; hipStream_t stream = nullptr; uint shardRank = 0, shardCount = 1;
    hipStream_t streams[PT_PIPELINE_BATCHES] = {}; WaveCounters* hostCounters = nullptr; bool serialKernels = false;
    uint tailBelow = PT_TAIL_PATHS, tailDefer = 0, fusedTraversal = PT_FUSED_TRAVERSAL; bool compactPool = PT_COMPACT_POOL != 0, firstVertexInPlace = PT_FIRST_VERTEX_IN_PLACE != 0;
    std::string lastError;
    std::vector<uint> indices; std::vector<float> positions; std::vector<ptk::float2> uvs; std::vector<uint> normals, tangents;
    std::vector<GeometryDesc> geometries; std::vector<MeshDesc> meshes; std::vector<InstanceDesc> instances;
    std::vector<ptk::PTMaterialData> materials; std::vector<HostTexture> textures; HostTexture envTex; bool envEnabled = false;
    float3x4 envToWorld, envToLocal; ptk::float3 envColorMul;
    uint envCubeDim = 2048; std::vector<ptk::EnvDirectionalLight> envDirLights, sceneDirLights; bool envCubeDirty = true;
    ptk::EnvCube envCube;
    std::vector<PolymorphicLightInfoFull> analyticLights;
    std::vector<SubInstanceData> subInstances; std::vector<ptk::uint2> subInstToInstGeom; std::vector<ptk::uint2> primInfo;
    std::vector<uint> subInstFirstPrim;
    std::vector<ptk::PolymorphicLightInfo> lights; std::vector<ptk::PolymorphicLightInfoEx> lightsEx; std::vector<uint> envLookup;
    uint envLookupDim = 0; uint numProxies = 0, envLightsBaked = 0;
    DevBuf<float> dLightW; DevBuf<uint> dProxyOffsets; void* dScanTemp = nullptr; size_t scanTempBytes = 0;
    DevBuf<uint> dIndices, dNormals, dTangents, dProxyCounters, dProxyIndices, dEnvLookup, dOwned, dQueue[2], dEmissiveList, dEmissiveOffsets;
    DevBuf<float> dPrevPositions; DevBuf<InstanceDesc> dPrevInstances; bool motionHistory = false, prevAllStale = false;
    std::vector<uint32_t> prevStaleRanges;
    DevBuf<float> dPositions; DevBuf<ptk::float2> dUvs; DevBuf<GeometryDesc> dGeometries; DevBuf<InstanceDesc> dInstances;
    DevBuf<SubInstanceData> dSubInstances;
    DevBuf<ptk::AlphaPlane> dAlphaPlanes; DevBuf<unsigned char> dAlphaPool; DevBuf<ptk::ShadeTri> dShadeTris;
    DevBuf<ptk::uint2> dSubInstToInstGeom, dPrimInfo; DevBuf<ptk::PTMaterialData> dMaterials; DevBuf<TexInfo> dTexInfos; DevBuf<ptk::float4> dTexels;
    bool skyEnabled = false; ptk::ProceduralSkyContext sky; DevBuf<ptk::float4> dSkyTex[4]; DevBuf<ptk::ProceduralSkyContext> dSky;
    DevBuf<ptk::uint2> dSkyLowRes;
    DevBuf<ptk::uint2> dEnvImageCube; uint envImageCubeDim = 0;
    DevBuf<ptk::uint2> dEnvCube, dEnvCubeSource; DevBuf<ptk::EnvDirectionalLight> dEnvDirLights; uint envCompression = 0;
    DevBuf<ptk::PolymorphicLightInfo> dLights; DevBuf<ptk::PolymorphicLightInfoEx> dLightsEx;
    DevBuf<uint> dLocalTable; uint localResX = 0, localResY = 0, localJitterX = 0, localJitterY = 0, localMaxLight = 0;
    float localRatio = 0.f, sscThreshold = 0.f; bool feedbackRequired = false;
    DevBuf<float> dFbWeight; DevBuf<uint> dFbCand; DevBuf<ptk::float4> dSq3; uint fbSamples = 0;
    ptk::LightFrustumBoost lightBoost = {}; bool weightsDirty = false;
    struct NeeAt {
        bool enabled = false; float globalFeedbackWeight = 0.75f, localRatio = 0.65f, sscThreshold = 0.3f, dropoff = 0.005f, intensityDeltaMul = 64.0f;
        bool preFilter = true;
        uint updateCounter = 0; float jitterF[2] = {0, 0}; uint jitter[2] = {0, 0}, prevJitter[2] = {0, 0};
        bool feedbackFilled = false, lastFeedbackAvailable = false; uint historicTotalLightCount = 0, W = 0, H = 0, nHist = 0;
        bool frameOpen = false, frameFeedbackAvailable = false, frameLocalAvailable = false, exportDepth = true; uint framePrevLightCount = 0;
        DevBuf<float> fbW, scW, blW, snapW, curW, histW; DevBuf<uint> fbC, scC, blC, snapC, local, counters;
        DevBuf<float> depth, histDepth; bool haveClip = false; float clipZ[4] = {0, 0, 0, 0}, clipW[4] = {0, 0, 0, 0};
        DevBuf<uint> xSend, xRecv; DevBuf<uint> xPixels; uint xW = 0, xH = 0;
        void reset() {
            W = H = 0; updateCounter = 0; jitterF[0] = jitterF[1] = 0; jitter[0] = jitter[1] = prevJitter[0] = prevJitter[1] = 0;
            feedbackFilled = lastFeedbackAvailable = false; frameOpen = false; exportDepth = true; historicTotalLightCount = 0; nHist = 0;
        }
        void free() {
            fbW.free(); scW.free(); blW.free(); snapW.free(); curW.free(); histW.free(); fbC.free(); scC.free(); blC.free(); snapC.free();
            local.free(); counters.free(); xSend.free(); xRecv.free(); xPixels.free(); depth.free(); histDepth.free();
        }
    } neeat;
    DevBuf<ptk::uint4> dS0, dS1, dS2, dS3, dS4, dHit, dS0b, dS1b, dS3b, dS4b, dHitb; DevBuf<ptk::float4> dSq0, dSq1, dSq2, dAccum, dScratch4;
    DevBuf<WaveCounters> dCounters; DevBuf<ptk::uint2> dTravSpill; DevBuf<ptk::TravTask> dTaskQ; DevBuf<uint> dTravCounts, dResolveList;
    DevBuf<unsigned long long> dBestKey;
    DevBuf<ptk::TravTask> dTaskQSh; DevBuf<uint> dResolveListSh; DevBuf<unsigned long long> dBestKeySh;
    std::vector<TexInfo> texInfos; TexInfo envTexInfo;
    BvhBuildBuffers bvh; bool bvhAllocated = false; uint numTris = 0; uint bvhBuilder = BVH_BUILDER_SAH;
    DeviceScene dsc;
    ptk::PtSettings S; ptk::PathTracerCameraData cam; uint width = 0, height = 0, accumCount = 0; std::vector<uint> owned;
    std::vector<std::vector<uint>> shardPixels;
    std::vector<float> hostRadiance; bool countersEnabled = false;
    bool geomDirty = true, lightsDirty = true, texDirty = true;
    double buildMs = 0, refitMs = 0, lightBakeMs = 0;
    uint poolCapacity = 0; size_t shadowCapacity = 0;
    DevBuf<uint> dSpHeader, dSpThroughput; DevBuf<ptk::StablePlane> dSpPlanes; DevBuf<ptk::uint2> dSpRadiance, dSpMotion;
    DevBuf<float> dSpDepth, dSpHitT; uint spW = 0, spH = 0; bool spGathered = false;
    DevBuf<ptk::uint4> dSpMark; DevBuf<ptk::float4> dSpNewL;
    DevBuf<float> dSpScratch; DevBuf<uint> dSpGatherSend, dSpGatherRecv, dSpGatherPixels; uint spGatherW = 0, spGatherH = 0;
    DevBuf<uint> dDnRRDiff, dDnRRSpec, dDnRRSpecMV; DevBuf<ptk::uint2> dDnRRNormal, dDnMotion; DevBuf<float> dDnViewZ, dDnRoughness;
    DevBuf<ptk::float4> dDnNormal, dDnDiff, dDnSpec;
    DevBuf<unsigned char> dDnDisocclusion, dDnHistoryClamp; uint dnW = 0, dnH = 0;
    uint spSampleBase = 0;
    DevBuf<ptk::float4> dRxHist[3][2][5], dRxOut[3][2], dRxGuide, dRxPing[2], dRxPong[2];
    uint rxW = 0, rxH = 0, rxSide[3] = {0, 0, 0}; bool rxHistory[3] = {false, false, false}, rxDenoised[3] = {false, false, false}; int dnPreparedPlane = -1;
    uint spFrameSerial = 0, rxFrameSerial[3] = {0, 0, 0};
    bool rxTiming = false; std::vector<float> rxPassMs; std::vector<hipEvent_t> rxEvents;
// ... 47 lines not shown
```

### rtxpt_amd/csrc/pt_frame.hip

```cpp
#include "pt_context.h"
#include <cstdio>
#include <cstdlib>
#include <cstring>

StablePlanesContext sp_context(pt_context* c, const PtStablePlanesParams* params) {
    ptk::StablePlanesParams prm;
    if (params) memcpy(&prm, params, sizeof(prm));
    else { memset(&prm, 0, sizeof(prm)); prm.activeStablePlaneCount = cStablePlaneCount; }
    StablePlanesContext sp; sp.C = ptk::SP_make_consts(prm, c->width, c->height, c->S.bounceCount);
    sp.B.Header = c->dSpHeader.p; sp.B.Planes = c->dSpPlanes.p; sp.B.StableRadiance = c->dSpRadiance.p; sp.B.Depth = c->dSpDepth.p;
    sp.B.SpecularHitT = c->dSpHitT.p; sp.B.MotionVectors = c->dSpMotion.p; sp.B.Throughput = c->dSpThroughput.p;
    return sp;
}

void add_frame_stats(PtFrameStats& t, const PtFrameStats& o) {
    t.extendRays += o.extendRays; t.shadowRays += o.shadowRays; t.hits += o.hits;
    t.nodeVisitsExtend += o.nodeVisitsExtend; t.triTestsExtend += o.triTestsExtend; t.nodeVisitsShadow += o.nodeVisitsShadow;
    t.triTestsShadow += o.triTestsShadow; t.leafVisitsExtend += o.leafVisitsExtend; t.waveItersExtend += o.waveItersExtend;
    t.leafVisitsShadow += o.leafVisitsShadow; t.waveItersShadow += o.waveItersShadow;
    for (int q = 0; q < 4; q++) t.extendPhaseCycles[q] += o.extendPhaseCycles[q];
    t.leafBlocksExtend += o.leafBlocksExtend; if (o.waveItersMaxExtend > t.waveItersMaxExtend) t.waveItersMaxExtend = o.waveItersMaxExtend;
    for (int q = 0; q < 16; q++) t.extendRayIterHist[q] += o.extendRayIterHist[q];
    for (uint q = 0; q < o.longRayCount && q < 32u && t.longRayCount < 32u; q++) { memcpy(t.longRays[t.longRayCount], o.longRays[q], 32); t.longRayCount++; }
    for (int q = 0; q < 8; q++) t.extendEvents[q] += o.extendEvents[q];
// ... 157 lines not shown
        PT_CHECK_HIP(c, c->dTaskQSh.resize((size_t)PT_PIPELINE_BATCHES * 2 * TASK_QUEUE_CAPACITY));
        for (uint b = 0; b < numBatches; b++) {
            RenderBatch& t = B[b]; const size_t sbase = (size_t)t.base * shadowPerPath;
            t.auxSh = shadow_aux(t);
            t.auxSh.taskQ[0] = c->dTaskQSh.p + (size_t)(2 * b) * TASK_QUEUE_CAPACITY; t.auxSh.taskQ[1] = t.auxSh.taskQ[0] + TASK_QUEUE_CAPACITY;
            t.auxSh.bestKey = c->dBestKeySh.p + sbase; t.auxSh.resolveList = c->dResolveListSh.p + sbase;
        }
        fused = true;
        return PT_OK;
    }
    int32_t enable_compact_pool() {
        PT_CHECK_HIP(c, c->dS0b.resize(c->poolCapacity)); PT_CHECK_HIP(c, c->dS1b.resize(c->poolCapacity)); PT_CHECK_HIP(c, c->dS3b.resize(c->poolCapacity));
        PT_CHECK_HIP(c, c->dS4b.resize(c->poolCapacity)); PT_CHECK_HIP(c, c->dHitb.resize(c->poolCapacity));
        for (uint b = 0; b < numBatches; b++) {
            RenderBatch& t = B[b]; t.compact = true; t.set = 0; t.poolSet[0] = t.pool;
            t.poolSet[1] = PathPool{c->dS0b.p + t.base, c->dS1b.p + t.base, t.pool.s2, c->dS3b.p + t.base, c->dS4b.p + t.base, c->dHitb.p + t.base, nullptr};
        }
        return PT_OK;
    }
    void enable_first_vertex_in_place() {
        for (uint b = 0; b < numBatches; b++) {
            RenderBatch& t = B[b]; t.firstInPlace = t.compact && !(tailBelow && t.total <= tailBelow);
            t.hwc->firstCamera.cam = t.k.cam; t.hwc->firstCamera.perPixelJitterAAScale = t.k.S.perPixelJitterAAScale;
        }
    }
    int32_t start() {
        for (uint b = 0; b < numBatches; b++) {
            RenderBatch& t = B[b];
            t.t0 = t.mark();
            PT_CHECK_HIP(c, hipMemcpyAsync(t.wc, t.hwc, sizeof(WaveCounters), hipMemcpyHostToDevice, t.st));
            if (!t.firstInPlace) launch_generate(t.k, t.pool, c->dOwned.p + t.pixFirst, t.numPix, first, count, 0u, t.total, t.queue[0], nullptr, t.st);
        }
        return PT_OK;
    }
    int32_t queue_pass(RenderBatch& t) {
        const uint nxt = t.cur ^ 1u;
        launch_pass_reset(t.aux.counts, &t.wc->extendCount[nxt], fused ? nullptr : &t.wc->shadowCount, t.st);
        if (tailBelow && t.active <= tailBelow && !t.afterTail) return queue_tail(t);
        t.afterTail = false; t.bound++; wavefrontPasses++;
        const size_t e0 = t.mark();
        PathPool pin = t.pool, pout = PathPool{};
        if (t.compact) { pin = t.poolSet[t.set]; pin.home = t.queue[t.cur]; pout = t.poolSet[t.set ^ 1u]; t.set ^= 1u; }
        const uint* countIn = &t.wc->extendCount[t.cur];
        const bool vertex0 = t.firstInPlace && t.iterations == 0u;
        const FirstVertex fv{c->dOwned.p + t.pixFirst, t.numPix, first, count};
        if (vertex0) launch_extend_first(t.k, pin, fv, countIn, t.active, t.wc, t.aux, t.st);
        else if (t.pendingShadow) {
            launch_trace_pair(t.sc, pin, t.queue[t.cur], countIn, t.active, t.sq, &t.wc->shadowCount, t.pendingShadow, t.wc, t.aux, t.auxSh, t.st);
            t.pendingShadow = 0;
        } else launch_extend(t.sc, pin, t.queue[t.cur], countIn, t.active, t.wc, c->countersEnabled, t.aux, t.st);
        const size_t e1 = t.mark(); t.span(e0, e1, 0, t.active);
        uint* classScratch = t.active >= PT_CLASSIFY_FROM ? reinterpret_cast<uint*>(t.aux.bestKey) : nullptr;
        launch_shade(t.k, pin, t.queue[t.cur], countIn, t.active, t.queue[nxt], &t.wc->extendCount[nxt], t.sq, t.wc, classScratch,
                     t.aux.counts + PASS_CLASS_OFFSET, t.st, pout, vertex0 ? &fv : nullptr);
        const size_t e2 = t.mark(); t.span(e1, e2, 1, t.active);
        t.extendRays += t.active;
        PT_CHECK_HIP(c, hipMemcpyAsync(t.hwc, t.wc, 16, hipMemcpyDeviceToHost, t.st));
        t.waiting = true;
        return PT_OK;
    }
    int32_t queue_tail(RenderBatch& t) {
        const uint nxt = t.cur ^ 1u;
        if (t.compact) {
            PathPool in = t.poolSet[t.set]; in.home = t.queue[t.cur];
            launch_uncompact(in, t.poolSet[t.set ^ 1u], &t.wc->extendCount[t.cur], t.active, t.st);
            t.pool = t.poolSet[t.set ^ 1u]; t.compact = false;
        }
        if (t.pendingShadow) {
            launch_shadow(t.sc, t.pool, t.sq, &t.wc->shadowCount, t.pendingShadow, t.wc, false, t.auxSh, t.st);
            PT_CHECK_HIP(c, hipMemsetAsync(&t.wc->shadowCount, 0, 4, t.st));
            t.pendingShadow = 0;
        }
        const size_t e0 = t.mark();
        launch_tail(t.k, t.pool, t.queue[t.cur], &t.wc->extendCount[t.cur], t.active, t.queue[nxt], &t.wc->extendCount[nxt], t.sq, t.wc, maxIter - t.bound,
                    c->tailDefer, t.aux.maxBlocks, t.st);
        const size_t e1 = t.mark(); t.span(e0, e1, 3, t.active);
        t.tailLaunches++; t.afterTail = true; t.inTail = true;
        PT_CHECK_HIP(c, hipMemcpyAsync(t.hwc, t.wc, 16, hipMemcpyDeviceToHost, t.st));
        t.waiting = true;
        return PT_OK;
    }
    int32_t finish_pass(RenderBatch& t, uint b) {
        t.waiting = false; t.inTail = false;
        const uint nxt = t.cur ^ 1u, nShadow = t.hwc->shadowCount;
        if (passLog) {
            uint pc[PASS_COUNTERS]; PT_CHECK_HIP(c, hipMemcpy(pc, t.aux.counts, sizeof(pc), hipMemcpyDeviceToHost));
            fprintf(stderr, "[pass log]   b%u pass %u: %u paths -> extend splits %u / %u / %u / %u sub-trees, %u rays resolved; %u visibility rays next\n",
                    b, t.iterations, t.active, pc[0], pc[1], pc[2], pc[3], pc[TRAV_RESOLVE], nShadow);
        }
        t.active = t.hwc->extendCount[nxt];
        if (fused && nShadow && live(t)) { t.pendingShadow = nShadow; t.shadowRays += nShadow; }
        else if (nShadow) {
            const size_t s0 = t.mark();
            launch_shadow(t.sc, t.pool, t.sq, &t.wc->shadowCount, nShadow, t.wc, c->countersEnabled, fused ? t.auxSh : shadow_aux(t), t.st);
            const size_t s1 = t.mark(); t.span(s0, s1, 2, nShadow);
            if (!shadowGroup) t.shadowRays += nShadow;
            if (fused) PT_CHECK_HIP(c, hipMemsetAsync(&t.wc->shadowCount, 0, 4, t.st));
        }
        t.cur = nxt; t.iterations++;
        return PT_OK;
    }
    int32_t lockstep() {
        static const uint freeRunBelow = []() {
            const char* e = getenv("MI355PT_FREE_RUN_BELOW"); return e ? (uint)strtoul(e, nullptr, 10) : (uint)PT_FREE_RUN_BELOW;
        }();
        for (;;) {
            bool freeRun = freeRunBelow != 0u && numBatches > 1u;
            for (uint b = 0; b < numBatches; b++) if (live(B[b]) && B[b].active >= freeRunBelow) freeRun = false;
            wavefrontPasses = 0;
            for (uint b = 0; b < numBatches; b++) {
                RenderBatch& t = B[b];
                if (t.waiting || !live(t)) continue;
                int32_t r = queue_pass(t); if (r != PT_OK) return r;
            }
            if (freeRun) return PT_OK;
            bool any = false;
            for (uint b = 0; b < numBatches; b++) {
                RenderBatch& t = B[b];
                if (!t.waiting) continue;
                if (t.inTail && wavefrontPasses && hipStreamQuery(t.st) == hipErrorNotReady) { any = true; continue; }
                PT_CHECK_HIP(c, hipStreamSynchronize(t.st));
                int32_t r = finish_pass(t, b); if (r != PT_OK) return r;
                if (live(t)) any = true;
            }
            if (!any) return PT_OK;
        }
    }
    int32_t free_run() {
        uint waiting = 0; for (uint b = 0; b < numBatches; b++) waiting += B[b].waiting ? 1u : 0u;
        while (waiting) {
            for (uint b = 0; b < numBatches; b++) {
                RenderBatch& t = B[b];
                if (!t.waiting || hipStreamQuery(t.st) == hipErrorNotReady) continue;
                PT_CHECK_HIP(c, hipStreamSynchronize(t.st));
                int32_t r = finish_pass(t, b); if (r != PT_OK) return r;
                waiting--;
                if (live(t)) { r = queue_pass(t); if (r != PT_OK) return r; waiting++; }
            }
        }
        return PT_OK;
    }
// ... 164 lines not shown
        launch_pass_reset(t.aux.counts, &t.wc->extendCount[nxt], &t.wc->shadowCount, t.st);
        launch_extend(t.sc, t.pool, t.queue[t.cur], &t.wc->extendCount[t.cur], t.active, t.wc, c->countersEnabled, t.aux, t.st);
        launch_sp_build_shade(t.k, sp, t.pool, t.queue[t.cur], &t.wc->extendCount[t.cur], t.active, t.queue[nxt], &t.wc->extendCount[nxt], sampleIndex, t.wc,
                              t.st);
        t.extendRays += t.active;
        PT_CHECK_HIP(c, hipMemcpyAsync(t.hwc, t.wc, 16, hipMemcpyDeviceToHost, t.st));
        PT_CHECK_HIP(c, hipStreamSynchronize(t.st));
        t.active = t.hwc->extendCount[nxt]; t.cur = nxt; t.iterations++;
    }
    return PT_OK;
}

}

extern "C" {

int32_t pt_render(pt_context* c, uint32_t first, uint32_t count, PtFrameStats* stats) {
    if (!c) return PT_ERROR_INVALID_ARGUMENT;
    if (!c->width) return fail(c, PT_ERROR_NOT_READY, "pt_resize first");
    if (!count) return PT_OK;
    (void)hipSetDevice(c->device);
    int r = prepare(c); if (r != PT_OK) return r;
    if (c->neeat.enabled && c->S.NEEEnabled && c->S.NEEFullSamples != 0u) {
        if (count > 1) return render_sample_by_sample(c, first, count, stats);
        r = neeat_exchange_feedback(c); if (r != PT_OK) return r;
        r = neeat_frame(c); if (r != PT_OK) return r;
    }
    const uint numOwned = (uint)c->owned.size();
    if ((unsigned long long)numOwned * count > 0xF0000000ull) return fail(c, PT_ERROR_INVALID_ARGUMENT, "too many paths in one pt_render call");
    const uint total = numOwned * count;
    if (stats) memset(stats, 0, sizeof(*stats));
    if (total == 0) { c->accumCount += count; return PT_OK; }
    const uint neeSamples = c->S.NEEFullSamples < 63u ? c->S.NEEFullSamples : 63u;
    const uint shadowGroup = (c->S.NEEEnabled && neeSamples > 1u) ? neeSamples : 0u;
    const uint shadowPerPath = shadowGroup ? shadowGroup : 1u;
    r = ensure_pool(c, total, shadowPerPath); if (r != PT_OK) return r;
    const bool feedback = c->feedbackRequired && c->S.NEEEnabled && neeSamples != 0u;
    r = prepare_neeat_layers(c, count, feedback, shadowGroup); if (r != PT_OK) return r;
    PathKernelContext k = kernel_context(c);
    if (neeSamples == 0u) k.S.NEEEnabled = 0;

    RenderFrame f{c, first, count, total, shadowGroup, shadowPerPath, feedback};
    r = f.setup(k); if (r != PT_OK) return r;
    if (f.numBatches > 1) PT_CHECK_HIP(c, hipStreamSynchronize(c->stream));
    Events frame; PT_CHECK_HIP(c, frame.record(c->stream));
    r = f.start(); if (r != PT_OK) return r;
    r = f.lockstep(); if (r != PT_OK) return r;
    r = f.free_run(); if (r != PT_OK) return r;
    f.accumulate();
    r = drain_frame(c, f.B, f.numBatches, frame); if (r != PT_OK) return r;
    c->accumCount += count;
    if (feedback) c->fbSamples = count;
    if (stats) f.harvest(*stats, frame.ms());
    if (f.passLog) f.log_passes();
    return check_frame_end(c, f.B, f.numBatches,
                           "pt_render: paths still alive at the pass bound (bounceCount + 2 + the nested-dielectric allowance): the bound must be raised");
}

int32_t pt_build_stable_planes(pt_context* c, uint32_t sampleIndex, const PtStablePlanesParams* params, PtFrameStats* stats) {
    if (!c || !params) return PT_ERROR_INVALID_ARGUMENT;
    if (!c->width) return fail(c, PT_ERROR_NOT_READY, "pt_resize first");
    (void)hipSetDevice(c->device);
    int r = prepare(c); if (r != PT_OK) return r;
    if (stats) memset(stats, 0, sizeof(*stats));
    const uint numOwned = (uint)c->owned.size();
    r = ensure_pool(c, numOwned ? numOwned : 1u, 1u); if (r != PT_OK) return r;
    r = ensure_stable_planes(c, ptk::GenericTSComputePlaneStride(c->width, c->height)); if (r != PT_OK) return r;
    const StablePlanesContext sp = sp_context(c, params);
    c->spGathered = false; c->spSampleBase = sampleIndex; c->dnPreparedPlane = -1; c->spFrameSerial++;
    if (!numOwned) return PT_OK;
    PathKernelContext k = kernel_context(c);
    Batch t; slice_batch(c, k, 0u, 1u, 1u, 1u, frame_shadow_queue(c, 0u), 0u, t);
    t.st = c->stream; t.hwc->extendCount[0] = t.active = t.total;
    Events frame; PT_CHECK_HIP(c, frame.record(t.st));
    PT_CHECK_HIP(c, hipMemcpyAsync(t.wc, t.hwc, sizeof(WaveCounters), hipMemcpyHostToDevice, t.st));
    launch_sp_generate(k, sp, t.pool, c->dOwned.p, numOwned, sampleIndex, t.queue[0], t.st);
    const uint depth = sp.C.maxStablePlaneVertexDepth, rejects = nested_dielectric_allowance(c->S);
    const uint maxIter = cStablePlaneCount * (depth + 2u + (c->S.nestedDielectricsQuality == 1 ? rejects * (depth + 1u) : rejects));
    r = build_passes(c, sp, sampleIndex, maxIter, t); if (r != PT_OK) return r;
    PT_CHECK_HIP(c, frame.record(t.st));
    PT_CHECK_HIP(c, hipMemcpyAsync(t.hwc, t.wc, sizeof(WaveCounters), hipMemcpyDeviceToHost, t.st));
    PT_CHECK_HIP(c, hipStreamSynchronize(t.st));
    PT_CHECK_HIP(c, hipGetLastError());
    if (stats) { *stats = batch_stats(t, 0u); stats->gpuMilliseconds = frame.ms(); }
    return check_frame_end(c, &t, 1u, "stable-plane build pass: paths still exploring after the iteration bound");
}

int32_t pt_fill_stable_planes(pt_context* c, uint32_t sampleIndex, const PtStablePlanesParams* params, PtFrameStats* stats) {
    if (!c || !params) return PT_ERROR_INVALID_ARGUMENT;
    if (!c->width) return fail(c, PT_ERROR_NOT_READY, "pt_resize first");
    if (!c->spW || c->spW != c->width || c->spH != c->height)
        return fail(c, PT_ERROR_NOT_READY, "no stable planes of this frame size yet: pt_build_stable_planes first");
    if (c->S.NEEEnabled && c->S.NEEFullSamples > 1u)
        return fail(c, PT_ERROR_INVALID_ARGUMENT, "the fill pass traces one full NEE sample per vertex (NEEFullSamples 0 or 1, the reference's default)");
    const bool feedback = c->neeat.enabled && c->feedbackRequired && c->S.NEEEnabled && c->S.NEEFullSamples != 0u;
    if (c->feedbackRequired && !c->neeat.enabled)
        return fail(c, PT_ERROR_INVALID_ARGUMENT, "the fill pass feeds NEE-AT's reservoirs only with the baker in the loop (pt_set_neeat, pt_realtime_frame): "
                                                  "switch the temporal feedback of pt_set_local_light_sampling off");
    if (feedback && (!c->neeat.fbW.p || c->neeat.W != c->width || c->neeat.H != c->height))
        return fail(c, PT_ERROR_NOT_READY, "NEE-AT: no baker frame of this size yet (pt_realtime_frame runs it)");
    (void)hipSetDevice(c->device);
    int r = prepare(c); if (r != PT_OK) return r;
    if (stats) memset(stats, 0, sizeof(*stats));
    const uint numOwned = (uint)c->owned.size();
    if (!numOwned) return PT_OK;
    r = ensure_pool(c, numOwned, 1u); if (r != PT_OK) return r;
// ... 22 lines not shown
```

### rtxpt_amd/csrc/pt_scene.h

```cpp
#pragma once
#include "pt_lights.h"
#include "pt_envcube.h"
#include "pt_sky.h"

namespace ptk {
#pragma clang force_cuda_host_device begin

enum : uint {
    PTMaterialFlags_UseSpecularGlossModel = 0x1, PTMaterialFlags_UseMetalRoughOrSpecularTexture = 0x4,
    PTMaterialFlags_UseBaseOrDiffuseTexture = 0x8, PTMaterialFlags_UseEmissiveTexture = 0x10, PTMaterialFlags_UseNormalTexture = 0x20,
    PTMaterialFlags_UseTransmissionTexture = 0x80, PTMaterialFlags_MetalnessInRedChannel = 0x100, PTMaterialFlags_ThinSurface = 0x200,
    PTMaterialFlags_EnableAsAnalyticLightProxy = 0x800, PTMaterialFlags_IgnoreMeshTangentSpace = 1u << 12, PTMaterialFlags_NestedPriorityShift = 28,
};
struct PTMaterialData {
    float3 BaseOrDiffuseColor; uint Flags;
    float3 SpecularColor; int _padding0;
    float3 EmissiveColor; float ShadowNoLFadeout;
    float Opacity, Roughness, Metalness, NormalTextureScale;
    float _padding1, AlphaCutoff, TransmissionFactor; uint BaseOrDiffuseTextureIndex;
    uint MetalRoughOrSpecularTextureIndex, EmissiveTextureIndex, NormalTextureIndex, OcclusionTextureIndex;
    uint TransmissionTextureIndex; float IoR, ThicknessFactor, DiffuseTransmissionFactor;
    float3 AttenuationColor; float AttenuationDistance;
};
static_assert(sizeof(PTMaterialData) == 128, "PTMaterialData must be 128 bytes");
// ... 16 lines not shown
    TriRecord t; t.x[0] = p0.x; t.x[1] = p1.x; t.x[2] = p2.x; t.prim = prim; t.y[0] = p0.y; t.y[1] = p1.y; t.y[2] = p2.y; t.flags = flags; t.z[0] = p0.z; t.z[1] = p1.z; t.z[2] = p2.z; t.pad = pad; return t;
}
static inline float3 tri_v0(const TriRecord& t) { return make_float3(t.x[0], t.y[0], t.z[0]); }
static inline float3 tri_v1(const TriRecord& t) { return make_float3(t.x[1], t.y[1], t.z[1]); }
static inline float3 tri_v2(const TriRecord& t) { return make_float3(t.x[2], t.y[2], t.z[2]); }
static inline void tri_bounds(const TriRecord& t, float3& mn, float3& mx) {
    mn = make_float3(fminf_(t.x[0], fminf_(t.x[1], t.x[2])), fminf_(t.y[0], fminf_(t.y[1], t.y[2])), fminf_(t.z[0], fminf_(t.z[1], t.z[2])));
    mx = make_float3(fmaxf_(t.x[0], fmaxf_(t.x[1], t.x[2])), fmaxf_(t.y[0], fmaxf_(t.y[1], t.y[2])), fmaxf_(t.z[0], fmaxf_(t.z[1], t.z[2])));
}
static_assert(sizeof(TriRecord) == 48, "TriRecord must be 48 bytes");
struct BvhNode { float3 lmin, lmax, rmin, rmax; uint left, right, _pad0, _pad1; };
static_assert(sizeof(BvhNode) == 64, "BvhNode must be 64 bytes");
#define PT_T8_LANES 2
#ifndef PT_BVH_MAX_LEAF
#define PT_BVH_MAX_LEAF 2
#endif
static const uint BVH_LEAF_BIT = 0x80000000u, BVH_EMPTY = 0xFFFFFFFFu, BVH_MAX_LEAF = PT_BVH_MAX_LEAF, BVH_STACK = 64;
struct Bvh8Child { uint ref, q0, q1; };
struct Bvh8Node { float ox, oy, oz; uint exps; Bvh8Child c[8]; uint _pad[4]; };
typedef uint u32x4 __attribute__((ext_vector_type(4)));
typedef uint u32x2 __attribute__((ext_vector_type(2)));
typedef float f32x2 __attribute__((ext_vector_type(2)));
struct __attribute__((packed, aligned(4))) u32x3p { uint x, y, z; };
typedef float f32x4 __attribute__((ext_vector_type(4)));
static_assert(sizeof(Bvh8Node) == 128, "Bvh8Node must be 128 bytes");
#ifndef PT_T8_CHUNK
#define PT_T8_CHUNK 32
#endif
#ifndef PT_BVH8_STACK
#define PT_BVH8_STACK 13
#endif
static const uint BVH8_STACK = PT_BVH8_STACK, BVH8_STACK_STRIDE = PT_BVH8_STACK + 1;
static const uint T8_BLOCK = 256, T8_CHUNK = PT_T8_CHUNK, T8_LANES = PT_T8_LANES, T8_GROUPS_PER_WAVE = 64 / PT_T8_LANES, T8_GROUPS_PER_BLOCK = T8_BLOCK / T8_LANES, T8_SPILL_DEPTH = 96;
#ifndef PT_T8_MAX_BLOCKS
#define PT_T8_MAX_BLOCKS (256 * 7 * 3)
#endif
static const uint T8_MAX_BLOCKS = PT_T8_MAX_BLOCKS;

struct AlphaRec { float2 t0, t1, t2; uint tex; float cutoff; uint wh; uint plane; uint fmt; uint _pad; };
static_assert(sizeof(AlphaRec) == 48, "AlphaRec must be 48 bytes");
struct AlphaPlane { uint wh, offset, fmt, _pad; };

struct TexInfo { uint w, h, mipLevels, _pad; unsigned long long base; uint mipOffset[16]; };

struct ShadeTri {
    uint instance, subInstance, triangleIndex, materialAndFlags;
    float3 p0, p1, p2;
    float2 t0, t1, t2;
    float3 n0, n1, n2;
    uint g0, g1, g2;
    uint _pad;
};
static_assert(sizeof(ShadeTri) == 128, "ShadeTri must be one 128-byte line");

struct DeviceScene {
    const uint* indices; const float* positions; const float2* uvs; const uint* normals; const uint* tangents;
    const float* prevPositions; const InstanceDesc* prevInstances;
    const GeometryDesc* geometries; const InstanceDesc* instances; const SubInstanceData* subInstances; const uint2* subInstToInstGeom;
    const PTMaterialData* materials; uint materialCount;
    const TexInfo* textures; const float4* texels;
    TexInfo envTex; uint envEnabled; float3x4 envToWorld, envToLocal; float3 envColorMultiplier;
    EnvCube envCube;
    const ProceduralSkyContext* sky;
    EnvCube skyLowRes;
    EnvCube envCubeSource;
    LightTable lights;
    const BvhNode* nodes; const Bvh8Node* nodes8; const TriRecord* tris; const uint2* primInfo; uint numTris, rootIsValid;
    const AlphaRec* alphaRecs;
    const AlphaPlane* alphaPlanes; const unsigned char* alphaPool;
    const ShadeTri* shadeTris;
    const uint* primToSlot;
    uint2* travSpill;
    const uint2* envImageCube; uint envImageCubeDim, _padEnvImageCube;
};

struct HitInfo { float t; uint prim; float u, v; };
struct TravTask { uint tag, ref, tbits, _pad; };
struct TravTaskOut { TravTask* tasks; uint* count; uint capacity; };

static inline const float4& tex_texel(const DeviceScene& sc, const TexInfo& t, uint mip, int x, int y) {
    uint mw = t.w >> mip; if (mw < 1u) mw = 1u;
    uint mh = t.h >> mip; if (mh < 1u) mh = 1u;
    int xi = x, yi = y;
    if (xi < 0) xi += (int)mw; else if (xi >= (int)mw) xi -= (int)mw;
    if (yi < 0) yi += (int)mh; else if (yi >= (int)mh) yi -= (int)mh;
    xi = xi < 0 ? 0 : (xi >= (int)mw ? (int)mw - 1 : xi);
    yi = yi < 0 ? 0 : (yi >= (int)mh ? (int)mh - 1 : yi);
    return sc.texels[t.base + t.mipOffset[mip] + (unsigned long long)yi * mw + (uint)xi];
}
static inline float wrap_texel_npot(float x, float side) {
    const float r = fmaf(-floorf(x / side), side, x);
    return r - floorf(r / side) * side;
}
static inline float4 sample_bilinear(const DeviceScene& sc, const TexInfo& t, uint mip, float2 uv) {
    uint mw = t.w >> mip; if (mw < 1u) mw = 1u;
    uint mh = t.h >> mip; if (mh < 1u) mh = 1u;
    float fx = uv.x * (float)mw - 0.5f, fy = uv.y * (float)mh - 0.5f;
    float flx = floorf(fx), fly = floorf(fy);
    float ax = fx - flx, ay = fy - fly;
    const float fmw = (float)mw, fmh = (float)mh;
    if (((mw & (mw - 1u)) | (mh & (mh - 1u))) == 0u) { flx = flx - floorf(flx * asfloat(0x7F000000u - asuint(fmw))) * fmw; fly = fly - floorf(fly * asfloat(0x7F000000u - asuint(fmh))) * fmh; }
    else { flx = wrap_texel_npot(flx, fmw); fly = wrap_texel_npot(fly, fmh); }
    int x0 = (int)flx, y0 = (int)fly;
    float4 a = lerp4(tex_texel(sc, t, mip, x0, y0), tex_texel(sc, t, mip, x0 + 1, y0), ax);
    float4 b = lerp4(tex_texel(sc, t, mip, x0, y0 + 1), tex_texel(sc, t, mip, x0 + 1, y0 + 1), ax);
    return lerp4(a, b, ay);
// ... 149 lines not shown
```

### rtxpt_amd/csrc/pt_wavefront.h

```cpp
#pragma once
#include "pt_path.h"
#include "pt_neeat.h"
#include "pt_tonemap.h"
#include <hip/hip_runtime.h>

namespace ptk {

struct PathPool { uint4* s0; uint4* s1; uint4* s2; uint4* s3; uint4* s4; uint4* hit;
    const uint* home; };
struct ShadowQueue { float4* q0; float4* q1; float4* q2; uint group;
    float4* q3; float* fbTotalWeight; uint* fbCandidates; uint fbWidth, fbPlane, fbSampleFirst; };
struct FirstVertex { const uint* ownedPixels; uint numOwned, sampleFirst, spp; };
struct FirstVertexCamera { PathTracerCameraData cam; float perPixelJitterAAScale, _pad[3]; };
struct WaveCounters {
    uint extendCount[2]; uint shadowCount; uint overflow;
    unsigned long long hits, nodeVisitsExt, triTestsExt, nodeVisitsSh, triTestsSh, leafVisitsExt, itersExt, leafVisitsSh, itersSh, phaseCycExt[4], leafBlocksExt, eventsExt[8], itersMaxExt, rayIterHistExt[16]; uint longRayCount, _padLong; float longRays[32][8];
    unsigned long long shadowValid;
    unsigned long long tailExtendRays, tailShadowRays;
    unsigned long long tailHandedBack[3];
    FirstVertexCamera firstCamera;
};

static const uint TRAV_COUNTERS = 5, TRAV_RESOLVE = 4, PASS_COUNTERS = 16, PASS_SHADOW_OFFSET = 5, PASS_CLASS_OFFSET = 10;
struct TravAux { TravTask* taskQ[2]; uint* counts; uint taskCap; unsigned long long* bestKey; uint* resolveList; const uint* primToSlot; uint maxBlocks; };

void launch_generate(const PathKernelContext& k, PathPool pool, const uint* ownedPixels, uint numOwned, uint sampleFirst, uint spp, uint first, uint n, uint* queue, uint* countPtr, hipStream_t st);
void launch_extend(const DeviceScene& sc, PathPool pool, const uint* queue, const uint* countPtr, uint count, WaveCounters* wc, bool counters, TravAux aux, hipStream_t st, bool ranged = false);
void launch_extend_first(const PathKernelContext& k, PathPool pool, FirstVertex fv, const uint* countPtr, uint count, WaveCounters* wc, TravAux aux, hipStream_t st);
void launch_shade(const PathKernelContext& k, PathPool pool, const uint* queueIn, const uint* countInPtr, uint countIn, uint* queueOut, uint* countOutPtr,
                  ShadowQueue sq, WaveCounters* wc, uint* classScratch, uint* classCount, hipStream_t st, PathPool outPool = PathPool{},
                  const FirstVertex* fv = nullptr);
void launch_uncompact(PathPool in, PathPool out, const uint* countPtr, uint count, hipStream_t st);
void launch_classify(PathPool pool, const uint* queueIn, const uint* countInPtr, uint countIn, uint* classScratch, uint* classCount, hipStream_t st);
void launch_shadow(const DeviceScene& sc, PathPool pool, ShadowQueue sq, const uint* countPtr, uint count, WaveCounters* wc, bool counters, TravAux aux, hipStream_t st);
void launch_trace_pair(const DeviceScene& sc, PathPool pool, const uint* queue, const uint* extCountPtr, uint extCount, ShadowQueue sq, uint* shCountPtr, uint shCount, WaveCounters* wc, TravAux auxE, TravAux auxS, hipStream_t st);
void launch_tail(const PathKernelContext& k, PathPool pool, const uint* queueIn, const uint* countInPtr, uint countIn, uint* queueOut, uint* countOutPtr, ShadowQueue sq, WaveCounters* wc, uint maxBounces, uint deferIters , uint maxBlocks, hipStream_t st);
void launch_pass_reset(uint* passCounters, uint* nextCount, uint* shadowCount, hipStream_t st);
void launch_accumulate(PathPool pool, const uint* ownedPixels, uint numOwned, uint spp, float4* accum, uint accumCountBase, uint width, hipStream_t st);
void launch_trace_probe(const DeviceScene& sc, const float4* rays, uint n, float4* outClosest, uint* outVisible, uint* overflow, hipStream_t st);
void launch_pack(const float4* accum, const uint* ownedPixels, uint numOwned, uint width, float4* dst, hipStream_t st);
void launch_unpack(float4* accum, const uint* pixels, uint num, uint width, const float4* src, hipStream_t st);
void launch_pack_feedback(const float* fbW, const uint* fbC, const float* depth, const uint* pixels, uint num, uint width, uint* dst, hipStream_t st);
void launch_unpack_feedback(float* fbW, uint* fbC, float* depth, const uint* pixels, uint num, uint width, const uint* src, hipStream_t st);
void launch_env_cube_bake(const DeviceScene& sc, const EnvDirectionalLight* lights, uint nLights, uint2* texels, const EnvCube& cube, hipStream_t st);
void launch_env_cube_compress(uint2* texels, const EnvCube& cube, uint quality, hipStream_t st);
void launch_env_importance(const DeviceScene& sc, uint dim, uint sx, uint sy, float4* out, hipStream_t st);
void launch_bake_emissive(const DeviceScene& sc, const uint* subInstList, const uint* subInstTriOffset, uint numEmissiveSubInst, uint totalTris, uint lightBase,
                          PolymorphicLightInfo* lights, PolymorphicLightInfoEx* lightsEx, hipStream_t st);
void launch_light_weights(const PolymorphicLightInfo* lights, const PolymorphicLightInfoEx* lightsEx, uint n, float* w, const LightFrustumBoost& boost, hipStream_t st);
void launch_light_proxy_counts(const float* w, uint n, float* sum, uint budget, bool uniform, uint maxPerLight, uint* counts, const uint* usage, uint totalMaxFeedbackCount, float globalFeedbackUseWeight, hipStream_t st);
void launch_neeat_boost_weights(const float* base, const float* hist, uint nHist, uint n, float mul, float* cur, hipStream_t st);
void launch_neeat_begin(const NeeAtFrame& F, float* snapW, uint* snapC, bool preFilter, uint totalThreads, hipStream_t st);
void launch_neeat_end(const NeeAtFrame& F, hipStream_t st);
void launch_light_proxy_fill(const uint* counts, const uint* offsets, uint n, uint* proxies, uint capacity, hipStream_t st);
void launch_tonemap(const float4* accum, uint num, const ToneMapParams& p, uint* outRgba8, hipStream_t st);
void launch_average_log_luminance(const float4* accum, uint W, uint H, float* scratch, float** result, hipStream_t st);
void launch_probe(const PathKernelContext& k, int kind, const void* dIn, void* dOut, uint n, hipStream_t st);

}
```

### rtxpt_amd/csrc/pt_wavefront.hip

```cpp
#include "pt_wavefront.h"
#include "pt_traverse8.h"
#include "pt_traverse8p.h"
#include "pt_wavefront_device.h"
#include <cstdlib>
#define T8_TRAVERSE traverse8_pairs

namespace ptk {

#ifndef T8_CHUNKS_PER_WAVE_MIN
#define T8_CHUNKS_PER_WAVE_MIN 1
#endif
#ifndef T8_SHORT_TAIL_BELOW
#define T8_SHORT_TAIL_BELOW 32768u
#endif
#ifndef T8_TASK_BLOCKS_N
#define T8_TASK_BLOCKS_N 512
#endif

__global__ void __launch_bounds__(256) k_generate(PathKernelContext k, PathPool pool, const uint* __restrict__ ownedPixels, uint numOwned, uint sampleFirst, uint spp, uint first, uint n, uint* __restrict__ queue, uint* countPtr) {
    const uint t = blockIdx.x * 256u + threadIdx.x;
    if (t >= n) return;
    const uint i = first + t;
    uint px, sample; first_vertex_of(FirstVertex{ownedPixels, numOwned, sampleFirst, spp}, i, px, sample);
    PathState p = k.generate(px >> 16, px & 0xFFFFu, sample);
// ... 74 lines not shown
        TravTask t = tasks[pad ? 0u : j];
        if (pad) t.tbits = 0x7F800000u;
        uint4 a = pool.s0[t.tag], b = pool.s1[t.tag];
        o = make_float3(asfloat(a.x), asfloat(a.y), asfloat(a.z)); d = make_float3(asfloat(b.x), asfloat(b.y), asfloat(b.z));
        unsigned long long key = aux.bestKey[t.tag];
        tmin = 0.0f; tmax = kMaxRayTravel; bestT0 = __uint_as_float((uint)(key >> 32)); bestPrim0 = (uint)key;
        startRef = (__uint_as_float(t.tbits) <= bestT0) ? t.ref : BVH_EMPTY;
        return t.tag;
    };
    auto commit = [&](uint p, const HitInfo& h) { atomicMin(&aux.bestKey[p], t8_hit_key(h.t, h.prim)); };
    auto publish = [&](uint p, float bestT, uint bestPrim) { if (bestPrim != 0xFFFFFFFFu) atomicMin(&aux.bestKey[p], t8_hit_key(bestT, bestPrim)); };
    T8_TRAVERSE<false, false, true, true, !FINAL>(sc, per * T8_CHUNK, T8_CHUNK, stack, rayBuf, nullptr, fetch, commit, publish, TravTaskOut{aux.taskQ[IN ^ 1], &aux.counts[FINAL ? STAGE : STAGE + 1], FINAL ? 0u : aux.taskCap}, ctr, &wc->overflow, vBlock, vGrid);
}
template <int STAGE, bool FINAL = (STAGE == 3)>
__global__ void __launch_bounds__(T8_BLOCK, T8_EXTEND_MIN_BLOCKS) k_extend_tasks(DeviceScene sc, PathPool pool, WaveCounters* wc, TravAux aux) {
    __shared__ uint2 stack[T8_GROUPS_PER_BLOCK * BVH8_STACK_STRIDE];
    __shared__ uint rayBuf[T8_TASKBUF_WORDS];
    t8_extend_tasks_body<STAGE, FINAL>(sc, pool, wc, aux, stack, rayBuf, blockIdx.x, gridDim.x);
}

__device__ __forceinline__ void t8_resolve_extend_body(const DeviceScene& sc, const PathPool& pool, const TravAux& aux, const uint vBlock, const uint vGrid) {
    const uint n = aux.counts[TRAV_RESOLVE];
    for (uint i = vBlock * 256u + threadIdx.x; i < n; i += vGrid * 256u) {
        uint p = aux.resolveList[i];
        unsigned long long key = aux.bestKey[p];
        uint prim = (uint)key;
        uint4 out = make_uint4((uint)(key >> 32), prim, 0u, 0u);
        if (prim != 0xFFFFFFFFu) {
            uint4 a = pool.s0[p], b = pool.s1[p];
            float3 o = make_float3(asfloat(a.x), asfloat(a.y), asfloat(a.z)), d = make_float3(asfloat(b.x), asfloat(b.y), asfloat(b.z));
            float t, u = 0.f, v = 0.f;
            const TriRecord tr = sc.tris[aux.primToSlot[prim]]; (void)intersect_tri_wt(tri_v0(tr), tri_v1(tr), tri_v2(tr), o, d, 0.0f, kMaxRayTravel, t, u, v);
            out.z = asuint(u); out.w = asuint(v);
        }
        pool.hit[p] = out;
    }
}
__global__ void __launch_bounds__(256) k_resolve_extend(DeviceScene sc, PathPool pool, TravAux aux) { t8_resolve_extend_body(sc, pool, aux, blockIdx.x, gridDim.x); }

#ifndef PT_SHADE_BLOCK
#define PT_SHADE_BLOCK 256
#endif
#ifndef PT_SHADE_MIN_BLOCKS
#define PT_SHADE_MIN_BLOCKS 1
#endif
#ifndef PT_SHADE_PROBE
#define PT_SHADE_PROBE 0
#endif
#ifndef PT_SHADE_CLASSES
#define PT_SHADE_CLASSES 1
#endif

#define PT_CLASSIFY_ITEMS 4u
template <bool UNIFORM = false>
__global__ void __launch_bounds__(1024) k_classify(PathPool pool, const uint* __restrict__ queueIn, const uint* __restrict__ countInPtr, uint* __restrict__ classQ, uint* __restrict__ classCount, uint uniformFlags) {
    __shared__ uint waveCnt[PT_CLASSIFY_ITEMS][16][3]; __shared__ uint blockBase[3];
    const uint count = *countInPtr, wave = threadIdx.x >> 6, lane = threadIdx.x & 63u;
    uint p[PT_CLASSIFY_ITEMS], cls[PT_CLASSIFY_ITEMS]; unsigned long long mine[PT_CLASSIFY_ITEMS];
#pragma unroll
    for (uint j = 0; j < PT_CLASSIFY_ITEMS; j++) {
        const uint i = (blockIdx.x * PT_CLASSIFY_ITEMS + j) * 1024u + threadIdx.x;
        p[j] = 0u; cls[j] = 3u;
        if (i < count) {
            p[j] = pool.home ? i : queueIn[i];
            const uint prim = reinterpret_cast<const uint*>(pool.hit)[4u * (size_t)p[j] + 1u], flags = UNIFORM ? uniformFlags : reinterpret_cast<const uint*>(pool.s4)[4u * (size_t)p[j] + 2u];
            cls[j] = (prim == 0xFFFFFFFFu) ? 2u : (((flags >> kVertexIndexBitCount) & PF_terminateAtNextBounce) ? 1u : 0u);
        }
        const unsigned long long m0 = __builtin_amdgcn_ballot_w64(cls[j] == 0u), m1 = __builtin_amdgcn_ballot_w64(cls[j] == 1u), m2 = __builtin_amdgcn_ballot_w64(cls[j] == 2u);
        if (lane == 0u) { waveCnt[j][wave][0] = (uint)__popcll(m0); waveCnt[j][wave][1] = (uint)__popcll(m1); waveCnt[j][wave][2] = (uint)__popcll(m2); }
        mine[j] = cls[j] == 0u ? m0 : (cls[j] == 1u ? m1 : m2);
    }
    __syncthreads();
    if (threadIdx.x < 3u) {
        uint tot = 0;
        for (uint j = 0; j < PT_CLASSIFY_ITEMS; j++) for (uint w = 0; w < 16u; w++) { const uint c = waveCnt[j][w][threadIdx.x]; waveCnt[j][w][threadIdx.x] = tot; tot += c; }
        blockBase[threadIdx.x] = tot ? atomicAdd(&classCount[threadIdx.x], tot) : 0u;
    }
    __syncthreads();
#pragma unroll
    for (uint j = 0; j < PT_CLASSIFY_ITEMS; j++) {
        if (cls[j] > 2u) continue;
        const uint rank = blockBase[cls[j]] + waveCnt[j][wave][cls[j]] + (uint)__popcll(mine[j] & ((1ull << lane) - 1ull));
        classQ[cls[j] == 0u ? rank : (cls[j] == 1u ? count - 1u - rank : count + rank)] = p[j];
    }
}

template <bool MULTI, class PKC, bool NEEAT, bool COMPACT = false, bool FIRST = false>
__global__ void __launch_bounds__(PT_SHADE_BLOCK, PT_SHADE_MIN_BLOCKS) k_shade(PKC k, PathPool pool, const uint* __restrict__ queueIn, const uint* __restrict__ countInPtr,
                                               uint* __restrict__ queueOut, uint* countOutPtr, ShadowQueue sq, WaveCounters* wc, const uint* __restrict__ classCount, PathPool outPool, FirstVertex fv) {
    static_assert(!FIRST || (COMPACT && !MULTI && !NEEAT), "vertex 0 in place: the compacted pool of a composed frame");
    static_assert(!COMPACT || !PT_SHADE_PROBE, "the PT_SHADE_PROBE timing builds do not know the compacted pool: take the COMPACT launch out of launch_shade and run with MI355PT_COMPACT_POOL=0");
    const uint count = *countInPtr;
    uint i = blockIdx.x * (uint)PT_SHADE_BLOCK + threadIdx.x;
    bool inRange = i < count;
    bool alive = false; bool isHit = false; uint p = 0, hp = 0;
    ShadowRequest req; req.valid = false;
    PathState cpath;
    if (COMPACT) __builtin_memset(&cpath, 0, sizeof(cpath));
    if (inRange) {
        if (classCount) {
            const uint nGo = classCount[0], nEnd = classCount[1];
            p = queueIn[i < nGo ? i : (i < nGo + nEnd ? count - 1u - (i - nGo) : count + (i - nGo - nEnd))];
        } else p = COMPACT ? i : queueIn[i];
        hp = (COMPACT && !FIRST) ? pool.home[p] : p;
        uint4 hr = pool.hit[p];
        HitInfo h; h.t = asfloat(hr.x); h.prim = hr.y; h.u = asfloat(hr.z); h.v = asfloat(hr.w);
#if PT_SHADE_PROBE
        PathState path = load_path(pool, p);
#if PT_SHADE_PROBE == 1
        if (h.prim != 0xFFFFFFFFu) { isHit = true; path.sceneLength += h.t; } path.terminate();
#elif PT_SHADE_PROBE == 2
        if (h.prim != 0xFFFFFFFFu) { isHit = true; SurfaceData sfd = k.loadSurface(h.prim, h.u, h.v, path.dir, path.rayCone); path.origin = sfd.shadingData.posW + sfd.shadingData.N * sfd.bsdf.data.roughness + sfd.bsdf.data.diffuse + sfd.shadingData.T; } path.terminate();
#endif
        store_path(pool, p, path);
        alive = path.isActive();
#else
        if (COMPACT && FIRST) {
            uint px, sample; first_vertex_of(fv, p, px, sample);
            const PathFirstVertexIO<PKC> io{k, px, sample};
            if (h.prim == 0xFFFFFFFFu) { cpath = io.load_all(); k.template HandleMiss<NEEAT>(cpath, cpath.dir, kMaxRayTravel); }
            else { isHit = true; cpath = io.load_first(); k.template HandleHit<false, NEEAT>(cpath, h, req, nullptr, io); }
            alive = cpath.isActive();
            pool.s2[hp] = make_uint4(cpath.pack23[0], cpath.pack23[1], cpath.pack45[0], cpath.pack45[1]);
        }
        else if (COMPACT) {
            const PathCompactIO io{pool, p, hp};
            if (h.prim == 0xFFFFFFFFu) { cpath = io.load_all(); k.template HandleMiss<NEEAT>(cpath, cpath.dir, kMaxRayTravel); }
            else { isHit = true; cpath = io.load_first(); k.template HandleHit<false, NEEAT>(cpath, h, req, nullptr, io); }
            alive = cpath.isActive();
            pool.s2[hp] = make_uint4(cpath.pack23[0], cpath.pack23[1], cpath.pack45[0], cpath.pack45[1]);
        }
        else if (h.prim == 0xFFFFFFFFu) { PathState path = load_path(pool, p); k.template HandleMiss<NEEAT>(path, path.dir, kMaxRayTravel); store_path(pool, p, path); alive = path.isActive(); }
        else {
            isHit = true;
            const PathPoolIO io{pool, p};
            PathState path = io.load_first();
            if (MULTI) { ShadowSink sink{sq.q0, sq.q1, sq.q2, &wc->shadowCount, &wc->shadowValid, p}; k.template HandleHit<true, NEEAT>(path, h, req, &sink, io); }
            else k.template HandleHit<false, NEEAT>(path, h, req, nullptr, io);
            alive = path.isActive();
#ifdef PT_SHADE_PHASE_PROBE
            for (int q = 1; q < 6; q++) wave_add64(io.tk[q] ? (unsigned long long)(uint)(io.tk[q] - io.tk[q - 1 - (io.tk[q - 1] ? 0 : 1)]) : 0ull, &wc->eventsExt[q - 1]);
#endif
        }
#endif
    }
    __shared__ uint sCnt[PT_SHADE_BLOCK / 64][2]; __shared__ uint sBase[2];
    const uint wave = threadIdx.x >> 6, lane = threadIdx.x & 63u;
    const unsigned long long mAlive = __builtin_amdgcn_ballot_w64(alive), mReq = __builtin_amdgcn_ballot_w64(!MULTI && req.valid);
    if (lane == 0u) { sCnt[wave][0] = (uint)__popcll(mAlive); sCnt[wave][1] = (uint)__popcll(mReq); }
    __syncthreads();
    if (threadIdx.x < 2u) {
        uint tot = 0; for (uint w = 0; w < (uint)(PT_SHADE_BLOCK / 64); w++) { const uint c = sCnt[w][threadIdx.x]; sCnt[w][threadIdx.x] = tot; tot += c; }
        sBase[threadIdx.x] = tot ? atomicAdd(threadIdx.x == 0u ? countOutPtr : &wc->shadowCount, tot) : 0u;
    }
    __syncthreads();
    const unsigned long long below = (1ull << lane) - 1ull;
    if (alive) {
        const uint slot = sBase[0] + sCnt[wave][0] + (uint)__popcll(mAlive & below);
        queueOut[slot] = hp;
        if (COMPACT) {
            outPool.s0[slot] = make_uint4(asuint(cpath.origin.x), asuint(cpath.origin.y), asuint(cpath.origin.z), cpath.id);
            outPool.s1[slot] = make_uint4(asuint(cpath.dir.x), asuint(cpath.dir.y), asuint(cpath.dir.z), asuint(cpath.sceneLength));
            outPool.s3[slot] = make_uint4(cpath.interiorList.slots[0], cpath.interiorList.slots[1], cpath.packedCounters, cpath.rayCone.widthSpreadAngleFP16);
            outPool.s4[slot] = make_uint4(cpath.pack0, cpath.pack1, cpath.flagsAndVertexIndex, cpath.sampleIndex);
        }
    }
    if (!MULTI && req.valid) {
        const uint sslot = sBase[1] + sCnt[wave][1] + (uint)__popcll(mReq & below);
        sq.q0[sslot] = make_float4(req.origin.x, req.origin.y, req.origin.z, req.tmax);
        sq.q1[sslot] = make_float4(req.dir.x, req.dir.y, req.dir.z, asfloat(hp));
        sq.q2[sslot] = make_float4(req.radiance.x, req.radiance.y, req.radiance.z, 0.f);
        if (NEEAT && sq.q3) sq.q3[sslot] = make_float4(req.fbWeight, req.fbRandom, asfloat(req.fbLight), asfloat(req.rrFix));
    }
    if (classCount) { if (blockIdx.x == 0u && threadIdx.x == 0u) atomicAdd(&wc->hits, (unsigned long long)classCount[0] + classCount[1]); }
    else wave_add64(isHit ? 1ull : 0ull, &wc->hits);
}

__device__ __forceinline__ void shadow_mark_visible(ShadowQueue sq, uint i) { reinterpret_cast<float*>(sq.q2 + i)[3] = 1.0f; }
template <bool GROUPED>
__device__ __forceinline__ void shadow_visible(PathPool pool, ShadowQueue sq, uint i) {
    if (GROUPED) { shadow_mark_visible(sq, i); return; }
    float4 r = sq.q2[i];
    uint p = asuint(sq.q1[i].w);
    uint4 c = pool.s2[p];
    uint pack45[2] = {c.z, c.w};
    PathKernelContext::ResolveShadow(pack45, make_float3(r.x, r.y, r.z));
    c.z = pack45[0]; c.w = pack45[1];
    pool.s2[p] = c;
    if (sq.q3) {
        const float4 f = sq.q3[i];
        const uint light = asuint(f.z), fix = asuint(f.w);
        if (light != RTXPT_INVALID_LIGHT_INDEX) {
            uint4 e = pool.s4[p];
            const uint id = pool.s0[p].w, slot = (e.w - sq.fbSampleFirst) * sq.fbPlane + (id & 0xFFFFu) * sq.fbWidth + (id >> 16);
            float total = sq.fbTotalWeight[slot]; uint cand = sq.fbCandidates[slot];
            LightFeedbackReservoir_Add(total, cand, f.y, light & ~LFR_SCREEN_SPACE_COHERENT_FLAG, f.x, (light & LFR_SCREEN_SPACE_COHERENT_FLAG) != 0u);
            sq.fbTotalWeight[slot] = total; sq.fbCandidates[slot] = cand;
            if (fix & 1u) {
                const uint bit = (uint)PF_terminateAtNextBounce << kVertexIndexBitCount;
                if (fix & 2u) e.z |= bit; else { e.z &= ~bit; e.y = (e.y & 0xFFFF0000u) | (fix >> 16); }
                pool.s4[p] = e;
            }
        }
    }
}

template <bool COUNT>
__device__ __forceinline__ void t8_shadow_body(const DeviceScene& sc, const ShadowQueue& sq, const uint count, WaveCounters* wc, const TravAux& aux, const uint rpc,
                                               uint2* stack, uint* rayBuf, const uint vBlock, const uint vGrid) {
    Traverse8Counters ctr; t8_counters_init(ctr);
    auto fetch = [&](uint i, float3& o, float3& d, float& tmin, float& tmax, uint& startRef, float& bestT0, uint& bestPrim0) -> uint {
        float4 a = sq.q0[i], b = sq.q1[i];
        o = make_float3(a.x, a.y, a.z); d = make_float3(b.x, b.y, b.z); tmin = 0.0f; tmax = a.w; startRef = 0u; bestT0 = a.w; bestPrim0 = 0xFFFFFFFFu;
        return i;
    };
    auto commit = [&](uint i, const HitInfo& h) { if (h.prim == 0xFFFFFFFFu) shadow_mark_visible(sq, i); };
    auto publish = [&](uint i, float, uint) { aux.bestKey[i] = 0ull; aux.resolveList[atomicAdd(&aux.counts[TRAV_RESOLVE], 1u)] = i; };
    T8_TRAVERSE<true, COUNT, false, false, true>(sc, count, rpc, stack, rayBuf, nullptr, fetch, commit, publish, TravTaskOut{aux.taskQ[0], &aux.counts[0], aux.taskCap}, ctr, &wc->overflow, vBlock, vGrid);
    if (COUNT) { wave_add64(ctr.nodeVisits, &wc->nodeVisitsSh); wave_add64(ctr.triTests, &wc->triTestsSh); wave_add64(ctr.leafVisits, &wc->leafVisitsSh); wave_add64(ctr.iters, &wc->itersSh); }
}
template <bool COUNT>
__global__ void __launch_bounds__(T8_BLOCK, COUNT ? 1 : T8_SHADOW_MIN_WAVES) k_shadow(DeviceScene sc, ShadowQueue sq, const uint* __restrict__ countPtr, WaveCounters* wc, TravAux aux, uint rpc) {
    __shared__ uint2 stack[T8_GROUPS_PER_BLOCK * BVH8_STACK_STRIDE];
    __shared__ uint rayBuf[T8_RAYBUF_WORDS];
    t8_shadow_body<COUNT>(sc, sq, *countPtr, wc, aux, rpc, stack, rayBuf, blockIdx.x, gridDim.x);
}

// ... 395 lines not shown
void launch_extend_first(const PathKernelContext& k, PathPool pool, FirstVertex fv, const uint* countPtr, uint count, WaveCounters* wc, TravAux aux, hipStream_t st) {
    const uint rpc = rays_per_chunk(count);
    const uint g = grid_for(count, (T8_BLOCK / 64u) * rpc * T8_CHUNKS_PER_WAVE_MIN, (aux.maxBlocks && aux.maxBlocks < T8_MAX_BLOCKS) ? aux.maxBlocks : T8_MAX_BLOCKS);
    hipLaunchKernelGGL(k_extend_first, dim3(g), dim3(T8_BLOCK), 0, st, k.sc, pool, fv, countPtr, wc, aux, rpc);
    hipLaunchKernelGGL(k_first_split_rays, dim3(T8_RESOLVE_BLOCKS), dim3(256), 0, st, k, pool, fv, aux);
    launch_extend_stragglers(k.sc, pool, count, wc, aux, st);
}
void launch_extend(const DeviceScene& sc, PathPool pool, const uint* queue, const uint* countPtr, uint count, WaveCounters* wc, bool counters, TravAux aux, hipStream_t st, bool ranged) {
    const uint rpc = rays_per_chunk(count);
    uint g = grid_for(count, (T8_BLOCK / 64u) * rpc * T8_CHUNKS_PER_WAVE_MIN, (aux.maxBlocks && aux.maxBlocks < T8_MAX_BLOCKS) ? aux.maxBlocks : T8_MAX_BLOCKS);
    if (ranged) { if (counters) hipLaunchKernelGGL((k_extend<true, true>), dim3(g), dim3(T8_BLOCK), 0, st, sc, pool, queue, countPtr, wc, aux, rpc);
                  else hipLaunchKernelGGL((k_extend<false, true>), dim3(g), dim3(T8_BLOCK), 0, st, sc, pool, queue, countPtr, wc, aux, rpc); }
    else if (counters) hipLaunchKernelGGL((k_extend<true>), dim3(g), dim3(T8_BLOCK), 0, st, sc, pool, queue, countPtr, wc, aux, rpc);
    else hipLaunchKernelGGL((k_extend<false>), dim3(g), dim3(T8_BLOCK), 0, st, sc, pool, queue, countPtr, wc, aux, rpc);
    launch_extend_stragglers(sc, pool, count, wc, aux, st);
}
static void launch_extend_stragglers(const DeviceScene& sc, PathPool pool, uint count, WaveCounters* wc, TravAux aux, hipStream_t st) {
    if (count <= T8_SHORT_TAIL_BELOW) {
        hipLaunchKernelGGL((k_extend_tasks<0>), dim3(T8_TASK_BLOCKS), dim3(T8_BLOCK), 0, st, sc, pool, wc, aux);
        hipLaunchKernelGGL((k_extend_tasks<1, true>), dim3(T8_TASK_BLOCKS), dim3(T8_BLOCK), 0, st, sc, pool, wc, aux);
        hipLaunchKernelGGL(k_resolve_extend, dim3(T8_RESOLVE_BLOCKS), dim3(256), 0, st, sc, pool, aux);
        return;
    }
    hipLaunchKernelGGL((k_extend_tasks<0>), dim3(T8_TASK_BLOCKS), dim3(T8_BLOCK), 0, st, sc, pool, wc, aux);
    hipLaunchKernelGGL((k_extend_tasks<1>), dim3(T8_TASK_BLOCKS), dim3(T8_BLOCK), 0, st, sc, pool, wc, aux);
    hipLaunchKernelGGL((k_extend_tasks<2>), dim3(T8_TASK_BLOCKS), dim3(T8_BLOCK), 0, st, sc, pool, wc, aux);
    hipLaunchKernelGGL((k_extend_tasks<3>), dim3(T8_TASK_BLOCKS), dim3(T8_BLOCK), 0, st, sc, pool, wc, aux);
    hipLaunchKernelGGL(k_resolve_extend, dim3(T8_RESOLVE_BLOCKS), dim3(256), 0, st, sc, pool, aux);
}
void launch_trace_pair(const DeviceScene& sc, PathPool pool, const uint* queue, const uint* extCountPtr, uint extCount, ShadowQueue sq, uint* shCountPtr, uint shCount, WaveCounters* wc, TravAux auxE, TravAux auxS, hipStream_t st) {
    const uint rpc = rays_per_chunk(extCount + shCount);
    const uint bound = (auxE.maxBlocks && auxE.maxBlocks < T8_MAX_BLOCKS) ? auxE.maxBlocks : T8_MAX_BLOCKS;
    uint gE = grid_for(extCount, (T8_BLOCK / 64u) * rpc * T8_CHUNKS_PER_WAVE_MIN, bound), gS = grid_for(shCount, (T8_BLOCK / 64u) * rpc * T8_CHUNKS_PER_WAVE_MIN, bound);
    if (gE + gS > bound) {
        uint s = (uint)(((unsigned long long)bound * shCount + (extCount + shCount) / 2u) / (extCount + shCount)); if (s < 1u) s = 1u; if (s > bound - 1u) s = bound - 1u;
        if (s > gS) s = gS;
        uint e = bound - s; if (e > gE) { e = gE; s = (bound - e < gS) ? bound - e : gS; }
        gE = e; gS = s;
    }
    hipLaunchKernelGGL(k_trace_pair, dim3(gE + gS), dim3(T8_BLOCK), 0, st, sc, pool, queue, extCountPtr, sq, shCountPtr, wc, auxE, auxS, rpc, rpc, gE);
    const dim3 tg(2u * T8_TASK_BLOCKS), tb(T8_BLOCK);
    if (extCount <= T8_SHORT_TAIL_BELOW && shCount <= T8_SHORT_TAIL_BELOW) {
        hipLaunchKernelGGL((k_tasks_pair<0>), tg, tb, 0, st, sc, pool, sq, wc, auxE, auxS);
        hipLaunchKernelGGL((k_tasks_pair<1, true>), tg, tb, 0, st, sc, pool, sq, wc, auxE, auxS);
    } else {
        hipLaunchKernelGGL((k_tasks_pair<0>), tg, tb, 0, st, sc, pool, sq, wc, auxE, auxS);
        hipLaunchKernelGGL((k_tasks_pair<1>), tg, tb, 0, st, sc, pool, sq, wc, auxE, auxS);
        hipLaunchKernelGGL((k_tasks_pair<2>), tg, tb, 0, st, sc, pool, sq, wc, auxE, auxS);
        hipLaunchKernelGGL((k_tasks_pair<3>), tg, tb, 0, st, sc, pool, sq, wc, auxE, auxS);
    }
    hipLaunchKernelGGL(k_resolve_pair, dim3(T8_RESOLVE_BLOCKS + shadow_resolve_grid(shCount)), dim3(256), 0, st, sc, pool, sq, auxE, auxS, shCountPtr, shCount, T8_RESOLVE_BLOCKS);
}
void launch_classify(PathPool pool, const uint* queueIn, const uint* countInPtr, uint countIn, uint* classScratch, uint* classCount, hipStream_t st) {
    hipLaunchKernelGGL((k_classify<false>), dim3((countIn + 1024u * PT_CLASSIFY_ITEMS - 1u) / (1024u * PT_CLASSIFY_ITEMS)), dim3(1024), 0, st, pool, queueIn, countInPtr, classScratch, classCount, 0u);
}
void launch_shade(const PathKernelContext& k, PathPool pool, const uint* queueIn, const uint* countInPtr, uint countIn, uint* queueOut, uint* countOutPtr, ShadowQueue sq, WaveCounters* wc,
                  uint* classScratch, uint* classCount, hipStream_t st, PathPool outPool, const FirstVertex* fv) {
    const FirstVertex fv0 = fv ? *fv : FirstVertex{nullptr, 0u, 0u, 0u};
    const dim3 g((countIn + PT_SHADE_BLOCK - 1) / PT_SHADE_BLOCK), b(PT_SHADE_BLOCK);
    if (PT_SHADE_CLASSES && classScratch) {
        const dim3 cg((countIn + 1024u * PT_CLASSIFY_ITEMS - 1u) / (1024u * PT_CLASSIFY_ITEMS));
        if (fv) hipLaunchKernelGGL((k_classify<true>), cg, dim3(1024), 0, st, pool, queueIn, countInPtr, classScratch, classCount, k.generateState(0u, 0u, 0u).flagsAndVertexIndex);
        else hipLaunchKernelGGL((k_classify<false>), cg, dim3(1024), 0, st, pool, queueIn, countInPtr, classScratch, classCount, 0u);
        queueIn = classScratch;
    } else classCount = nullptr;
    const bool neeat = k.sc.lights.LocalSamplingBuffer != nullptr || k.sc.lights.TemporalFeedbackRequired != 0u;
#define PT_LAUNCH_SHADE(MULTI, PKC, CTX) do { if (neeat) hipLaunchKernelGGL((k_shade<MULTI, PKC, true>), g, b, 0, st, CTX, pool, queueIn, countInPtr, queueOut, countOutPtr, sq, wc, classCount, outPool, fv0); \
                                              else if (pool.home && !MULTI && fv) hipLaunchKernelGGL((k_shade<false, PKC, false, true, true>), g, b, 0, st, CTX, pool, queueIn, countInPtr, queueOut, countOutPtr, sq, wc, classCount, outPool, fv0); \
                                              else if (pool.home && !MULTI) hipLaunchKernelGGL((k_shade<false, PKC, false, true>), g, b, 0, st, CTX, pool, queueIn, countInPtr, queueOut, countOutPtr, sq, wc, classCount, outPool, fv0); \
                                              else hipLaunchKernelGGL((k_shade<MULTI, PKC, false>), g, b, 0, st, CTX, pool, queueIn, countInPtr, queueOut, countOutPtr, sq, wc, classCount, outPool, fv0); } while (0)
    if (k.S.useFp16Types) {
        static_assert(sizeof(PathKernelContextT<true>) == sizeof(PathKernelContext), "the two lp builds share one context layout");
        PathKernelContextT<true> k16; __builtin_memcpy(&k16, &k, sizeof(k16));
        if (sq.group) PT_LAUNCH_SHADE(true, PathKernelContextT<true>, k16); else PT_LAUNCH_SHADE(false, PathKernelContextT<true>, k16);
    } else {
        if (sq.group) PT_LAUNCH_SHADE(true, PathKernelContext, k); else PT_LAUNCH_SHADE(false, PathKernelContext, k);
    }
#undef PT_LAUNCH_SHADE
}
void launch_shadow(const DeviceScene& sc, PathPool pool, ShadowQueue sq, const uint* countPtr, uint count, WaveCounters* wc, bool counters, TravAux aux, hipStream_t st) {
    const uint rpc = rays_per_chunk(count);
    uint g = grid_for(count, (T8_BLOCK / 64u) * rpc * T8_CHUNKS_PER_WAVE_MIN, (aux.maxBlocks && aux.maxBlocks < T8_MAX_BLOCKS) ? aux.maxBlocks : T8_MAX_BLOCKS);
    if (counters && !sq.group) hipLaunchKernelGGL((k_shadow<true>), dim3(g), dim3(T8_BLOCK), 0, st, sc, sq, countPtr, wc, aux, rpc);
    else hipLaunchKernelGGL((k_shadow<false>), dim3(g), dim3(T8_BLOCK), 0, st, sc, sq, countPtr, wc, aux, rpc);
    hipLaunchKernelGGL((k_shadow_tasks<0>), dim3(T8_TASK_BLOCKS), dim3(T8_BLOCK), 0, st, sc, sq, wc, aux);
    if (count <= T8_SHORT_TAIL_BELOW) hipLaunchKernelGGL((k_shadow_tasks<1, true>), dim3(T8_TASK_BLOCKS), dim3(T8_BLOCK), 0, st, sc, sq, wc, aux);
    else {
    hipLaunchKernelGGL((k_shadow_tasks<1>), dim3(T8_TASK_BLOCKS), dim3(T8_BLOCK), 0, st, sc, sq, wc, aux);
    hipLaunchKernelGGL((k_shadow_tasks<2>), dim3(T8_TASK_BLOCKS), dim3(T8_BLOCK), 0, st, sc, sq, wc, aux);
    hipLaunchKernelGGL((k_shadow_tasks<3>), dim3(T8_TASK_BLOCKS), dim3(T8_BLOCK), 0, st, sc, sq, wc, aux);
    }
    if (sq.group) hipLaunchKernelGGL((k_resolve_shadow<true>), dim3(T8_RESOLVE_BLOCKS), dim3(256), 0, st, pool, sq, aux, 0u);
    else hipLaunchKernelGGL((k_resolve_shadow<false>), dim3(shadow_resolve_grid(count)), dim3(256), 0, st, pool, sq, aux, count);
    if (sq.group) hipLaunchKernelGGL(k_resolve_nee, dim3(grid_for(count / sq.group, 256, 4096)), dim3(256), 0, st, pool, sq, countPtr);
}
__global__ void __launch_bounds__(64) k_pass_begin(uint* __restrict__ passCounters, uint* __restrict__ nextCount, uint* __restrict__ shadowCount) {
    if (threadIdx.x < PASS_COUNTERS) passCounters[threadIdx.x] = 0u;
    if (threadIdx.x == 32u) *nextCount = 0u;
    if (threadIdx.x == 33u && shadowCount) *shadowCount = 0u;
}
void launch_pass_reset(uint* passCounters, uint* nextCount, uint* shadowCount, hipStream_t st) { static_assert(PASS_COUNTERS <= 32u, "k_pass_begin"); hipLaunchKernelGGL(k_pass_begin, dim3(1), dim3(64), 0, st, passCounters, nextCount, shadowCount); }
__global__ void __launch_bounds__(256) k_uncompact(PathPool in, PathPool out, const uint* __restrict__ countPtr) {
    const uint i = blockIdx.x * 256u + threadIdx.x;
    if (i >= *countPtr) return;
    const uint hp = in.home[i];
    out.s0[hp] = in.s0[i]; out.s1[hp] = in.s1[i]; out.s3[hp] = in.s3[i]; out.s4[hp] = in.s4[i];
}
void launch_uncompact(PathPool in, PathPool out, const uint* countPtr, uint count, hipStream_t st) {
    if (count) hipLaunchKernelGGL(k_uncompact, dim3((count + 255u) / 256u), dim3(256), 0, st, in, out, countPtr);
}
void launch_accumulate(PathPool pool, const uint* ownedPixels, uint numOwned, uint spp, float4* accum, uint accumCountBase, uint width, hipStream_t st) {
    hipLaunchKernelGGL(k_accumulate, dim3((numOwned + 255) / 256), dim3(256), 0, st, pool, ownedPixels, numOwned, spp, accum, accumCountBase, width);
}
void launch_trace_probe(const DeviceScene& sc, const float4* rays, uint n, float4* outClosest, uint* outVisible, uint* overflow, hipStream_t st) {
    hipLaunchKernelGGL(k_trace_probe, dim3(grid_for(n, T8_BLOCK, T8_MAX_BLOCKS)), dim3(T8_BLOCK), 0, st, sc, rays, n, outClosest, outVisible, overflow);
}
__global__ void __launch_bounds__(256) k_pack_feedback(const float* __restrict__ fbW, const uint* __restrict__ fbC, const float* __restrict__ depth, const uint* __restrict__ pixels, uint num, uint width, uint* __restrict__ dst) {
    uint i = blockIdx.x * 256u + threadIdx.x; if (i >= num) return;
    const uint px = pixels[i], slot = (px & 0xFFFFu) * width + (px >> 16);
// ... 167 lines not shown
```

Before: 1874 Mrays/s.

## Drop terminating hits on non-emissive surfaces before shading via per-prim inert table

Builds a 2-bit-per-primitive table marking triangles whose material emits no light and is not an analytic light proxy, and, with nested dielectrics enabled, is thin. The classify pass uses it to move paths that terminate at this bounce and hit such a triangle into a fourth class that is never shaded. It still counts them as hits. The aim is to skip full shading work, including material fetch and NEE, for last-bounce hits that cannot add radiance. The cost is one extra table lookup per terminating path in classify and a rebuild of the table whenever geometry or lights change. It is correct only if such hits really contribute nothing, for example if no NEE or emission is done at the terminal vertex.

```diff
diff --git a/include/mi355pt_testhooks.h b/include/mi355pt_testhooks.h
--- a/include/mi355pt_testhooks.h
+++ b/include/mi355pt_testhooks.h
@@ -5,6 +5,7 @@
 extern "C" {
 #endif
 int32_t pt_probe(pt_context* ctx, int32_t kind, const void* in, size_t inBytes, void* out, size_t outBytes, uint32_t n);
+int32_t pt_get_inert_terminal(pt_context* ctx, uint32_t* numPrims, uint32_t* words, uint32_t capacityWords, uint64_t* lastDropped);
 #ifdef __cplusplus
 }
 #endif
diff --git a/rtxpt_amd/__init__.py b/rtxpt_amd/__init__.py
--- a/rtxpt_amd/__init__.py
+++ b/rtxpt_amd/__init__.py
@@ -35,7 +35,7 @@
     "pt_tonemap_upscaled", "pt_average_luminance_upscaled", "pt_upscale_tex_lod_bias",
     "pt_comm_unique_id", "pt_comm_init", "pt_comm_destroy", "pt_gather", "pt_shard_layout", "pt_gather_host", "pt_neeat_exchange_host",
 ]
-TEST_HOOK_EXPORTS = ["pt_probe"]
+TEST_HOOK_EXPORTS = ["pt_probe", "pt_get_inert_terminal"]
 
 
 class PtError(RuntimeError):
@@ -1260,3 +1260,13 @@
         out = np.zeros(out_shape, out_dtype)
         self._chk(self.L.pt_probe(self.h, kind, _p(inp), inp.nbytes, _p(out), out.nbytes, out_shape[0]), "pt_probe")
         return out
+
+    def inert_terminal(self):
+        if not self.test_hooks: raise RuntimeError("pt_get_inert_terminal is not part of the shipped library: PathTracer(test_hooks=True)")
+        n, dropped = ctypes.c_uint32(), ctypes.c_uint64()
+        self.L.pt_get_inert_terminal.argtypes = [ctypes.c_void_p, ctypes.c_void_p, ctypes.c_void_p, ctypes.c_uint32, ctypes.c_void_p]
+        self._chk(self.L.pt_get_inert_terminal(self.h, ctypes.byref(n), None, 0, ctypes.byref(dropped)), "pt_get_inert_terminal")
+        words = np.zeros((n.value + 15) // 16, np.uint32)
+        if n.value: self._chk(self.L.pt_get_inert_terminal(self.h, None, _p(words), words.size, None), "pt_get_inert_terminal")
+        prim = np.arange(n.value, dtype=np.uint32)
+        return ((words[prim // 16] >> (2 * (prim % 16))) & 3).astype(np.uint32), int(dropped.value)
diff --git a/rtxpt_amd/csrc/pt_api.hip b/rtxpt_amd/csrc/pt_api.hip
--- a/rtxpt_amd/csrc/pt_api.hip
+++ b/rtxpt_amd/csrc/pt_api.hip
@@ -210,7 +210,7 @@
     if (!c->bvhAllocated) { PT_CHECK_HIP(c, bvh_alloc(c->bvh, c->numTris)); c->bvhAllocated = true; }
     c->bvh.builder = c->bvhBuilder;
     { const char* e = getenv("MI355PT_REINSERT_PASSES"); c->bvh.riPasses = e ? (uint)atoi(e) : 12u; }
-    PT_CHECK_HIP(c, c->dShadeTris.resize(c->numTris));
+    PT_CHECK_HIP(c, c->dShadeTris.resize(c->numTris)); PT_CHECK_HIP(c, c->dInertBits.resize(inert_words(c->numTris)));
     if (!c->dTravSpill.p) PT_CHECK_HIP(c, c->dTravSpill.resize(PT_PIPELINE_BATCHES * (size_t)T8_MAX_BLOCKS * T8_GROUPS_PER_BLOCK * T8_SPILL_DEPTH));
     refresh_scene_view(c);
     hipEvent_t e0, e1; PT_CHECK_HIP(c, hipEventCreate(&e0)); PT_CHECK_HIP(c, hipEventCreate(&e1));
@@ -218,6 +218,7 @@
     PT_CHECK_HIP(c, bvh_build(c->bvh, c->dsc, c->numTris, st));
     PT_CHECK_HIP(c, hipEventRecord(e1, st));
     launch_shade_tris(c->dsc, 0u, c->numTris, c->dShadeTris.p, st);
+    launch_inert_bits(c->dsc, c->numTris, c->dInertBits.p, st);
     PT_CHECK_HIP(c, hipStreamSynchronize(st));
     float ms = 0; (void)hipEventElapsedTime(&ms, e0, e1); c->buildMs = ms; (void)hipEventDestroy(e0); (void)hipEventDestroy(e1);
     c->geomDirty = false; c->lightsDirty = true;
@@ -372,6 +373,7 @@
     } else { PT_CHECK_HIP(c, c->dLights.resize(1)); PT_CHECK_HIP(c, c->dLightsEx.resize(1)); }
     if (!keepEnv) PT_CHECK_HIP(c, c->dEnvLookup.upload(c->envLookup, c->stream));
     PT_CHECK_HIP(c, c->dSubInstances.upload(c->subInstances, c->stream));
+    if (c->dInertBits.p) launch_inert_bits(c->dsc, c->numTris, c->dInertBits.p, c->stream);
     PT_CHECK_HIP(c, hipEventRecord(e1, c->stream));
     PT_CHECK_HIP(c, hipStreamSynchronize(c->stream));
     float ms = 0; (void)hipEventElapsedTime(&ms, e0, e1); c->lightBakeMs = ms; (void)hipEventDestroy(e0); (void)hipEventDestroy(e1);
@@ -532,6 +534,7 @@
     { const char* e = getenv("MI355PT_COMPACT_POOL"); if (e) c->compactPool = atoi(e) != 0; }
     { const char* e = getenv("MI355PT_FIRST_VERTEX_IN_PLACE"); if (e) c->firstVertexInPlace = atoi(e) != 0; }
     { const char* e = getenv("MI355PT_FUSED_TRAVERSAL"); if (e) c->fusedTraversal = (uint)strtoul(e, nullptr, 10); }
+    { const char* e = getenv("MI355PT_DROP_INERT_TERMINAL"); if (e) c->dropInertTerminal = atoi(e) != 0; }
     { const char* e = getenv("MI355PT_TAIL_DEFER"); if (e) c->tailDefer = (uint)strtoul(e, nullptr, 10); }
     memset(&c->dsc, 0, sizeof(c->dsc)); memset(&c->cam, 0, sizeof(c->cam)); memset(&c->bvh, 0, sizeof(c->bvh));
     pt_default_settings(reinterpret_cast<::PtSettings*>(&c->S));
@@ -552,7 +555,7 @@
     if (c->bvhAllocated) bvh_free(c->bvh);
     c->dIndices.free(); c->dNormals.free(); c->dTangents.free(); c->dProxyCounters.free(); c->dProxyIndices.free(); c->dEnvLookup.free(); c->dOwned.free(); c->dQueue[0].free(); c->dQueue[1].free();
     c->dPrevPositions.free(); c->dPrevInstances.free(); c->dEmissiveList.free(); c->dEmissiveOffsets.free(); c->dPositions.free(); c->dUvs.free(); c->dGeometries.free(); c->dInstances.free(); c->dSubInstances.free(); c->dSubInstToInstGeom.free();
-    c->dPrimInfo.free(); c->dShadeTris.free(); c->dAlphaPlanes.free(); c->dAlphaPool.free(); c->dMaterials.free(); c->dTexInfos.free(); c->dTexels.free(); c->dEnvCube.free(); c->dEnvCubeSource.free(); c->dEnvImageCube.free(); c->dEnvDirLights.free(); c->dLights.free(); c->dLightsEx.free(); c->dS0.free(); c->dS1.free(); c->dS2.free(); c->dS3.free(); c->dS4.free();
+    c->dPrimInfo.free(); c->dShadeTris.free(); c->dInertBits.free(); c->dAlphaPlanes.free(); c->dAlphaPool.free(); c->dMaterials.free(); c->dTexInfos.free(); c->dTexels.free(); c->dEnvCube.free(); c->dEnvCubeSource.free(); c->dEnvImageCube.free(); c->dEnvDirLights.free(); c->dLights.free(); c->dLightsEx.free(); c->dS0.free(); c->dS1.free(); c->dS2.free(); c->dS3.free(); c->dS4.free();
     c->dHit.free(); c->dS0b.free(); c->dS1b.free(); c->dS3b.free(); c->dS4b.free(); c->dHitb.free(); c->dSq0.free(); c->dSq1.free(); c->dSq2.free(); c->dAccum.free(); c->dScratch4.free(); c->dCounters.free(); c->dTravSpill.free(); c->dTaskQ.free(); c->dTravCounts.free(); c->dResolveList.free(); c->dBestKey.free(); c->dResolveListSh.free(); c->dBestKeySh.free(); c->dTaskQSh.free();
     for (uint b = 1; b < PT_PIPELINE_BATCHES; b++) (void)hipStreamDestroy(c->streams[b]);
     (void)hipStreamDestroy(c->stream); (void)hipHostFree(c->hostCounters);
@@ -1436,6 +1439,18 @@
     di.free(); dout.free();
     return PT_OK;
 }
+int32_t pt_get_inert_terminal(pt_context* c, uint32_t* numPrims, uint32_t* words, uint32_t capacityWords, uint64_t* lastDropped) {
+    if (!c) return PT_ERROR_INVALID_ARGUMENT;
+    (void)hipSetDevice(c->device);
+    int r = prepare(c); if (r != PT_OK) return r;
+    if (numPrims) *numPrims = c->numTris;
+    if (lastDropped) *lastDropped = c->droppedTerminal;
+    if (words && c->numTris) {
+        if (capacityWords < inert_words(c->numTris)) return fail(c, PT_ERROR_INVALID_ARGUMENT, "inert-terminal table: (numPrims + 15) / 16 words");
+        PT_CHECK_HIP(c, hipMemcpy(words, c->dInertBits.p, 4 * (size_t)inert_words(c->numTris), hipMemcpyDeviceToHost));
+    }
+    return PT_OK;
+}
 #endif
 int32_t pt_shard_layout(uint32_t width, uint32_t height, uint32_t rank, uint32_t world, uint32_t* pixels, uint32_t capacity, uint32_t* count) {
     if (!width || !height || width > 65535 || height > 65535 || !world || rank >= world) return PT_ERROR_INVALID_ARGUMENT;
diff --git a/rtxpt_amd/csrc/pt_build.h b/rtxpt_amd/csrc/pt_build.h
--- a/rtxpt_amd/csrc/pt_build.h
+++ b/rtxpt_amd/csrc/pt_build.h
@@ -45,6 +45,7 @@
 void bvh_free(BvhBuildBuffers& b);
 hipError_t bvh_build(BvhBuildBuffers& b, const DeviceScene& sc, uint numTris, hipStream_t stream);
 void launch_shade_tris(const DeviceScene& sc, uint firstPrim, uint numTris, ShadeTri* out, hipStream_t stream);
+void launch_inert_bits(const DeviceScene& sc, uint numTris, uint* out, hipStream_t stream);
 hipError_t bvh_refit(BvhBuildBuffers& b, const DeviceScene& sc, uint numTris, hipStream_t stream);
 
 }
diff --git a/rtxpt_amd/csrc/pt_build.hip b/rtxpt_amd/csrc/pt_build.hip
--- a/rtxpt_amd/csrc/pt_build.hip
+++ b/rtxpt_amd/csrc/pt_build.hip
@@ -504,6 +504,15 @@
 }
 void launch_shade_tris(const DeviceScene& sc, uint firstPrim, uint numTris, ShadeTri* out, hipStream_t st) {
     if (numTris) hipLaunchKernelGGL(k_shade_tris, dim3((numTris + 255u) / 256u), dim3(256), 0, st, sc, firstPrim, numTris, out);
+}
+
+__global__ void __launch_bounds__(256) k_inert_bits(DeviceScene sc, uint numTris, uint* __restrict__ out) {
+    const uint w = blockIdx.x * 256u + threadIdx.x;
+    if (w >= inert_words(numTris)) return;
+    out[w] = inert_word(w, numTris, [&](uint p) -> const PTMaterialData& { return sc.materials[sc.subInstances[sc.primInfo[p].x].GlobalGeometryIndex_PTMaterialDataIndex & 0xFFFFu]; });
+}
+void launch_inert_bits(const DeviceScene& sc, uint numTris, uint* out, hipStream_t st) {
+    if (numTris) hipLaunchKernelGGL(k_inert_bits, dim3((inert_words(numTris) + 255u) / 256u), dim3(256), 0, st, sc, numTris, out);
 }
 
 __global__ void __launch_bounds__(256) k_wide_levels(const uint* __restrict__ levelIn, uint nIn, const uint* __restrict__ childL, const uint* __restrict__ childR,
diff --git a/rtxpt_amd/csrc/pt_context.h b/rtxpt_amd/csrc/pt_context.h
--- a/rtxpt_amd/csrc/pt_context.h
+++ b/rtxpt_amd/csrc/pt_context.h
@@ -68,6 +68,9 @@
 #ifndef PT_FIRST_VERTEX_IN_PLACE
 #define PT_FIRST_VERTEX_IN_PLACE 1
 #endif
+#ifndef PT_DROP_INERT_TERMINAL
+#define PT_DROP_INERT_TERMINAL 1
+#endif
 #ifndef PT_FREE_RUN_BELOW
 #define PT_FREE_RUN_BELOW (1u << 22)
 #endif
@@ -80,6 +83,7 @@
     int device = 0; hipStream_t stream = nullptr; uint shardRank = 0, shardCount = 1;
     hipStream_t streams[PT_PIPELINE_BATCHES] = {}; WaveCounters* hostCounters = nullptr; bool serialKernels = false;
     uint tailBelow = PT_TAIL_PATHS, tailDefer = 0, fusedTraversal = PT_FUSED_TRAVERSAL; bool compactPool = PT_COMPACT_POOL != 0, firstVertexInPlace = PT_FIRST_VERTEX_IN_PLACE != 0;
+    bool dropInertTerminal = PT_DROP_INERT_TERMINAL != 0; unsigned long long droppedTerminal = 0;
     std::string lastError;
     std::vector<uint> indices; std::vector<float> positions; std::vector<ptk::float2> uvs; std::vector<uint> normals, tangents;
     std::vector<GeometryDesc> geometries; std::vector<MeshDesc> meshes; std::vector<InstanceDesc> instances;
@@ -99,6 +103,7 @@
     DevBuf<float> dPositions; DevBuf<ptk::float2> dUvs; DevBuf<GeometryDesc> dGeometries; DevBuf<InstanceDesc> dInstances;
     DevBuf<SubInstanceData> dSubInstances;
     DevBuf<ptk::AlphaPlane> dAlphaPlanes; DevBuf<unsigned char> dAlphaPool; DevBuf<ptk::ShadeTri> dShadeTris;
+    DevBuf<uint> dInertBits;
     DevBuf<ptk::uint2> dSubInstToInstGeom, dPrimInfo; DevBuf<ptk::PTMaterialData> dMaterials; DevBuf<TexInfo> dTexInfos; DevBuf<ptk::float4> dTexels;
     bool skyEnabled = false; ptk::ProceduralSkyContext sky; DevBuf<ptk::float4> dSkyTex[4]; DevBuf<ptk::ProceduralSkyContext> dSky;
     DevBuf<ptk::uint2> dSkyLowRes;
diff --git a/rtxpt_amd/csrc/pt_frame.hip b/rtxpt_amd/csrc/pt_frame.hip
--- a/rtxpt_amd/csrc/pt_frame.hip
+++ b/rtxpt_amd/csrc/pt_frame.hip
@@ -233,7 +233,7 @@
         const size_t e1 = t.mark(); t.span(e0, e1, 0, t.active);
         uint* classScratch = t.active >= PT_CLASSIFY_FROM ? reinterpret_cast<uint*>(t.aux.bestKey) : nullptr;
         launch_shade(t.k, pin, t.queue[t.cur], countIn, t.active, t.queue[nxt], &t.wc->extendCount[nxt], t.sq, t.wc, classScratch,
-                     t.aux.counts + PASS_CLASS_OFFSET, t.st, pout, vertex0 ? &fv : nullptr);
+                     t.aux.counts + PASS_CLASS_OFFSET, t.st, pout, vertex0 ? &fv : nullptr, c->dropInertTerminal ? c->dInertBits.p : nullptr);
         const size_t e2 = t.mark(); t.span(e1, e2, 1, t.active);
         t.extendRays += t.active;
         PT_CHECK_HIP(c, hipMemcpyAsync(t.hwc, t.wc, 16, hipMemcpyDeviceToHost, t.st));
@@ -268,6 +268,9 @@
             uint pc[PASS_COUNTERS]; PT_CHECK_HIP(c, hipMemcpy(pc, t.aux.counts, sizeof(pc), hipMemcpyDeviceToHost));
             fprintf(stderr, "[pass log]   b%u pass %u: %u paths -> extend splits %u / %u / %u / %u sub-trees, %u rays resolved; %u visibility rays next\n",
                     b, t.iterations, t.active, pc[0], pc[1], pc[2], pc[3], pc[TRAV_RESOLVE], nShadow);
+            if (t.active >= PT_CLASSIFY_FROM)
+                fprintf(stderr, "[pass log]   b%u pass %u: classes %u continuing / %u terminating / %u misses, %u inert terminating hits dropped\n",
+                        b, t.iterations, pc[PASS_CLASS_OFFSET], pc[PASS_CLASS_OFFSET + 1], pc[PASS_CLASS_OFFSET + 2], pc[PASS_CLASS_OFFSET + 3]);
         }
         t.active = t.hwc->extendCount[nxt];
         if (fused && nShadow && live(t)) { t.pendingShadow = nShadow; t.shadowRays += nShadow; }
@@ -538,6 +541,7 @@
     c->accumCount += count;
     if (feedback) c->fbSamples = count;
     if (stats) f.harvest(*stats, frame.ms());
+    c->droppedTerminal = 0; for (uint b = 0; b < f.numBatches; b++) c->droppedTerminal += f.B[b].hwc->droppedTerminal;
     if (f.passLog) f.log_passes();
     return check_frame_end(c, f.B, f.numBatches,
                            "pt_render: paths still alive at the pass bound (bounceCount + 2 + the nested-dielectric allowance): the bound must be raised");
diff --git a/rtxpt_amd/csrc/pt_scene.h b/rtxpt_amd/csrc/pt_scene.h
--- a/rtxpt_amd/csrc/pt_scene.h
+++ b/rtxpt_amd/csrc/pt_scene.h
@@ -92,6 +92,24 @@
     uint _pad;
 };
 static_assert(sizeof(ShadeTri) == 128, "ShadeTri must be one 128-byte line");
+
+enum : uint { INERT_NO_LIGHT = 1u, INERT_THIN = 2u, INERT_PRIMS_PER_WORD = 16u };
+static inline uint inert_bits_of(const PTMaterialData& m) {
+    const bool noLight = m.EmissiveColor.x == 0.0f && m.EmissiveColor.y == 0.0f && m.EmissiveColor.z == 0.0f && (m.Flags & PTMaterialFlags_EnableAsAnalyticLightProxy) == 0u;
+    return (noLight ? (uint)INERT_NO_LIGHT : 0u) | ((m.Flags & PTMaterialFlags_ThinSurface) ? (uint)INERT_THIN : 0u);
+}
+static inline bool inert_when_terminal(uint bits, uint nestedDielectricsQuality) { return (bits & INERT_NO_LIGHT) != 0u && (nestedDielectricsQuality == 0u || (bits & INERT_THIN) != 0u); }
+static inline uint inert_words(uint numPrims) { return (numPrims + INERT_PRIMS_PER_WORD - 1u) / INERT_PRIMS_PER_WORD; }
+template <class MaterialOf> static inline uint inert_word(uint w, uint numPrims, MaterialOf materialOf) {
+    uint word = 0u;
+    for (uint j = 0; j < INERT_PRIMS_PER_WORD; j++) {
+        const uint p = w * INERT_PRIMS_PER_WORD + j;
+        if (p >= numPrims) break;
+        word |= inert_bits_of(materialOf(p)) << (2u * j);
+    }
+    return word;
+}
+static inline uint inert_bits_at(const uint* __restrict__ table, uint prim) { return (table[prim / INERT_PRIMS_PER_WORD] >> (2u * (prim % INERT_PRIMS_PER_WORD))) & 3u; }
 
 struct DeviceScene {
     const uint* indices; const float* positions; const float2* uvs; const uint* normals; const uint* tangents;
diff --git a/rtxpt_amd/csrc/pt_wavefront.h b/rtxpt_amd/csrc/pt_wavefront.h
--- a/rtxpt_amd/csrc/pt_wavefront.h
+++ b/rtxpt_amd/csrc/pt_wavefront.h
@@ -18,6 +18,7 @@
     unsigned long long shadowValid;
     unsigned long long tailExtendRays, tailShadowRays;
     unsigned long long tailHandedBack[3];
+    unsigned long long droppedTerminal;
     FirstVertexCamera firstCamera;
 };
 
@@ -29,7 +30,7 @@
 void launch_extend_first(const PathKernelContext& k, PathPool pool, FirstVertex fv, const uint* countPtr, uint count, WaveCounters* wc, TravAux aux, hipStream_t st);
 void launch_shade(const PathKernelContext& k, PathPool pool, const uint* queueIn, const uint* countInPtr, uint countIn, uint* queueOut, uint* countOutPtr,
                   ShadowQueue sq, WaveCounters* wc, uint* classScratch, uint* classCount, hipStream_t st, PathPool outPool = PathPool{},
-                  const FirstVertex* fv = nullptr);
+                  const FirstVertex* fv = nullptr, const uint* inertBits = nullptr);
 void launch_uncompact(PathPool in, PathPool out, const uint* countPtr, uint count, hipStream_t st);
 void launch_classify(PathPool pool, const uint* queueIn, const uint* countInPtr, uint countIn, uint* classScratch, uint* classCount, hipStream_t st);
 void launch_shadow(const DeviceScene& sc, PathPool pool, ShadowQueue sq, const uint* countPtr, uint count, WaveCounters* wc, bool counters, TravAux aux, hipStream_t st);
diff --git a/rtxpt_amd/csrc/pt_wavefront.hip b/rtxpt_amd/csrc/pt_wavefront.hip
--- a/rtxpt_amd/csrc/pt_wavefront.hip
+++ b/rtxpt_amd/csrc/pt_wavefront.hip
@@ -150,22 +150,26 @@
 #endif
 
 #define PT_CLASSIFY_ITEMS 4u
-template <bool UNIFORM = false>
-__global__ void __launch_bounds__(1024) k_classify(PathPool pool, const uint* __restrict__ queueIn, const uint* __restrict__ countInPtr, uint* __restrict__ classQ, uint* __restrict__ classCount, uint uniformFlags) {
-    __shared__ uint waveCnt[PT_CLASSIFY_ITEMS][16][3]; __shared__ uint blockBase[3];
+template <bool UNIFORM = false, bool DROP = false>
+__global__ void __launch_bounds__(1024) k_classify(PathPool pool, const uint* __restrict__ queueIn, const uint* __restrict__ countInPtr, uint* __restrict__ classQ, uint* __restrict__ classCount, uint uniformFlags,
+                                                   const uint* __restrict__ inertBits, uint nestedDielectricsQuality) {
+    static_assert(!(UNIFORM && DROP), "vertex 0 has no terminating paths");
+    __shared__ uint waveCnt[PT_CLASSIFY_ITEMS][16][4]; __shared__ uint blockBase[3];
     const uint count = *countInPtr, wave = threadIdx.x >> 6, lane = threadIdx.x & 63u;
     uint p[PT_CLASSIFY_ITEMS], cls[PT_CLASSIFY_ITEMS]; unsigned long long mine[PT_CLASSIFY_ITEMS];
 #pragma unroll
     for (uint j = 0; j < PT_CLASSIFY_ITEMS; j++) {
         const uint i = (blockIdx.x * PT_CLASSIFY_ITEMS + j) * 1024u + threadIdx.x;
-        p[j] = 0u; cls[j] = 3u;
+        p[j] = 0u; cls[j] = 4u;
         if (i < count) {
             p[j] = pool.home ? i : queueIn[i];
             const uint prim = reinterpret_cast<const uint*>(pool.hit)[4u * (size_t)p[j] + 1u], flags = UNIFORM ? uniformFlags : reinterpret_cast<const uint*>(pool.s4)[4u * (size_t)p[j] + 2u];
             cls[j] = (prim == 0xFFFFFFFFu) ? 2u : (((flags >> kVertexIndexBitCount) & PF_terminateAtNextBounce) ? 1u : 0u);
+            if (DROP && cls[j] == 1u && inert_when_terminal(inert_bits_at(inertBits, prim), nestedDielectricsQuality)) cls[j] = 3u;
         }
         const unsigned long long m0 = __builtin_amdgcn_ballot_w64(cls[j] == 0u), m1 = __builtin_amdgcn_ballot_w64(cls[j] == 1u), m2 = __builtin_amdgcn_ballot_w64(cls[j] == 2u);
         if (lane == 0u) { waveCnt[j][wave][0] = (uint)__popcll(m0); waveCnt[j][wave][1] = (uint)__popcll(m1); waveCnt[j][wave][2] = (uint)__popcll(m2); }
+        if (DROP) { const unsigned long long m3 = __builtin_amdgcn_ballot_w64(cls[j] == 3u); if (lane == 0u) waveCnt[j][wave][3] = (uint)__popcll(m3); }
         mine[j] = cls[j] == 0u ? m0 : (cls[j] == 1u ? m1 : m2);
     }
     __syncthreads();
@@ -173,6 +177,10 @@
         uint tot = 0;
         for (uint j = 0; j < PT_CLASSIFY_ITEMS; j++) for (uint w = 0; w < 16u; w++) { const uint c = waveCnt[j][w][threadIdx.x]; waveCnt[j][w][threadIdx.x] = tot; tot += c; }
         blockBase[threadIdx.x] = tot ? atomicAdd(&classCount[threadIdx.x], tot) : 0u;
+    } else if (DROP && threadIdx.x == 3u) {
+        uint tot = 0;
+        for (uint j = 0; j < PT_CLASSIFY_ITEMS; j++) for (uint w = 0; w < 16u; w++) tot += waveCnt[j][w][3];
+        if (tot) atomicAdd(&classCount[3], tot);
     }
     __syncthreads();
 #pragma unroll
@@ -198,8 +206,11 @@
     if (inRange) {
         if (classCount) {
             const uint nGo = classCount[0], nEnd = classCount[1];
-            p = queueIn[i < nGo ? i : (i < nGo + nEnd ? count - 1u - (i - nGo) : count + (i - nGo - nEnd))];
+            inRange = i < nGo + nEnd + classCount[2];
+            p = inRange ? queueIn[i < nGo ? i : (i < nGo + nEnd ? count - 1u - (i - nGo) : count + (i - nGo - nEnd))] : 0u;
         } else p = COMPACT ? i : queueIn[i];
+    }
+    if (inRange) {
         hp = (COMPACT && !FIRST) ? pool.home[p] : p;
         uint4 hr = pool.hit[p];
         HitInfo h; h.t = asfloat(hr.x); h.prim = hr.y; h.u = asfloat(hr.z); h.v = asfloat(hr.w);
@@ -270,7 +281,9 @@
         sq.q2[sslot] = make_float4(req.radiance.x, req.radiance.y, req.radiance.z, 0.f);
         if (NEEAT && sq.q3) sq.q3[sslot] = make_float4(req.fbWeight, req.fbRandom, asfloat(req.fbLight), asfloat(req.rrFix));
     }
-    if (classCount) { if (blockIdx.x == 0u && threadIdx.x == 0u) atomicAdd(&wc->hits, (unsigned long long)classCount[0] + classCount[1]); }
+    if (classCount) {
+        if (blockIdx.x == 0u && threadIdx.x == 0u) { const uint nDropped = classCount[3]; atomicAdd(&wc->hits, ((unsigned long long)classCount[0] + classCount[1]) + nDropped); if (nDropped) atomicAdd(&wc->droppedTerminal, (unsigned long long)nDropped); }
+    }
     else wave_add64(isHit ? 1ull : 0ull, &wc->hits);
 }
 
@@ -772,19 +785,21 @@
     hipLaunchKernelGGL(k_resolve_pair, dim3(T8_RESOLVE_BLOCKS + shadow_resolve_grid(shCount)), dim3(256), 0, st, sc, pool, sq, auxE, auxS, shCountPtr, shCount, T8_RESOLVE_BLOCKS);
 }
 void launch_classify(PathPool pool, const uint* queueIn, const uint* countInPtr, uint countIn, uint* classScratch, uint* classCount, hipStream_t st) {
-    hipLaunchKernelGGL((k_classify<false>), dim3((countIn + 1024u * PT_CLASSIFY_ITEMS - 1u) / (1024u * PT_CLASSIFY_ITEMS)), dim3(1024), 0, st, pool, queueIn, countInPtr, classScratch, classCount, 0u);
+    hipLaunchKernelGGL((k_classify<false>), dim3((countIn + 1024u * PT_CLASSIFY_ITEMS - 1u) / (1024u * PT_CLASSIFY_ITEMS)), dim3(1024), 0, st, pool, queueIn, countInPtr, classScratch, classCount, 0u, (const uint*)nullptr, 0u);
 }
 void launch_shade(const PathKernelContext& k, PathPool pool, const uint* queueIn, const uint* countInPtr, uint countIn, uint* queueOut, uint* countOutPtr, ShadowQueue sq, WaveCounters* wc,
-                  uint* classScratch, uint* classCount, hipStream_t st, PathPool outPool, const FirstVertex* fv) {
+                  uint* classScratch, uint* classCount, hipStream_t st, PathPool outPool, const FirstVertex* fv, const uint* inertBits) {
     const FirstVertex fv0 = fv ? *fv : FirstVertex{nullptr, 0u, 0u, 0u};
     const dim3 g((countIn + PT_SHADE_BLOCK - 1) / PT_SHADE_BLOCK), b(PT_SHADE_BLOCK);
+    const bool neeat = k.sc.lights.LocalSamplingBuffer != nullptr || k.sc.lights.TemporalFeedbackRequired != 0u;
     if (PT_SHADE_CLASSES && classScratch) {
         const dim3 cg((countIn + 1024u * PT_CLASSIFY_ITEMS - 1u) / (1024u * PT_CLASSIFY_ITEMS));
-        if (fv) hipLaunchKernelGGL((k_classify<true>), cg, dim3(1024), 0, st, pool, queueIn, countInPtr, classScratch, classCount, k.generateState(0u, 0u, 0u).flagsAndVertexIndex);
-        else hipLaunchKernelGGL((k_classify<false>), cg, dim3(1024), 0, st, pool, queueIn, countInPtr, classScratch, classCount, 0u);
+        const bool drop = inertBits && !neeat && k.sc.lights.DepthExport == nullptr;
+        if (fv) hipLaunchKernelGGL((k_classify<true>), cg, dim3(1024), 0, st, pool, queueIn, countInPtr, classScratch, classCount, k.generateState(0u, 0u, 0u).flagsAndVertexIndex, (const uint*)nullptr, 0u);
+        else if (drop) hipLaunchKernelGGL((k_classify<false, true>), cg, dim3(1024), 0, st, pool, queueIn, countInPtr, classScratch, classCount, 0u, inertBits, (uint)k.S.nestedDielectricsQuality);
+        else hipLaunchKernelGGL((k_classify<false>), cg, dim3(1024), 0, st, pool, queueIn, countInPtr, classScratch, classCount, 0u, (const uint*)nullptr, 0u);
         queueIn = classScratch;
     } else classCount = nullptr;
-    const bool neeat = k.sc.lights.LocalSamplingBuffer != nullptr || k.sc.lights.TemporalFeedbackRequired != 0u;
 #define PT_LAUNCH_SHADE(MULTI, PKC, CTX) do { if (neeat) hipLaunchKernelGGL((k_shade<MULTI, PKC, true>), g, b, 0, st, CTX, pool, queueIn, countInPtr, queueOut, countOutPtr, sq, wc, classCount, outPool, fv0); \
                                               else if (pool.home && !MULTI && fv) hipLaunchKernelGGL((k_shade<false, PKC, false, true, true>), g, b, 0, st, CTX, pool, queueIn, countInPtr, queueOut, countOutPtr, sq, wc, classCount, outPool, fv0); \
                                               else if (pool.home && !MULTI) hipLaunchKernelGGL((k_shade<false, PKC, false, true>), g, b, 0, st, CTX, pool, queueIn, countInPtr, queueOut, countOutPtr, sq, wc, classCount, outPool, fv0); \
```

After: 1913 Mrays/s, median of 6. +2.1%, better.
